# clintpgeorge/LDAGroupedGibbsSampler

Hardware: AMD Instinct MI355X
Metric: M tokens sampled/sec (whole node) per Gibbs sweep at K=100 (higher is better)
Workload: dtype f64

## Files before the change

### include/ggs_hip.h

```cpp
#ifndef GGS_HIP_H
#define GGS_HIP_H

#include <stdint.h>

#ifdef __cplusplus
extern "C" {
#endif

#define GGS_ABI_VERSION 6

typedef struct ggs_handle ggs_handle;

enum {
  GGS_OK = 0,
  GGS_ERR_NEGATIVE_COUNT = 1,
  GGS_ERR_INVALID_TOPIC = 2,
  GGS_ERR_RNG_EXHAUSTED = 3,
  GGS_ERR_BAD_ARG = 4,
  GGS_ERR_HIP = 5,
  GGS_ERR_STATE = 6,
  GGS_ERR_UNSUPPORTED = 7,
  GGS_ERR_INVARIANT = 8
};

// ... 47 lines not shown
  double exchange_ms;
  double exchange_rs_ms;
  double exchange_ag_ms;
} ggs_timings;

int ggs_create(const ggs_config *cfg, ggs_handle **out);
void ggs_destroy(ggs_handle *h);
const char *ggs_last_error(const ggs_handle *h);
int ggs_abi_version(void);
int ggs_set_stream(ggs_handle *h, void *hip_stream);

int ggs_set_corpus(ggs_handle *h, int64_t num_docs, const int64_t *doc_ptr ,
                   const int32_t *tokens , int64_t doc_base, int64_t tok_base);
int ggs_init_z_java_lcg(ggs_handle *h, int32_t seed);
int ggs_java_lcg_next_ints(int32_t seed, int32_t bound, int64_t n, int32_t *out);
int ggs_set_z(ggs_handle *h, const int32_t *z , int32_t redraw_phi);
int ggs_init_phi(ggs_handle *h);
int ggs_set_iteration(ggs_handle *h, int32_t iteration);
int ggs_get_iteration(const ggs_handle *h, int32_t *iteration);

int ggs_sweep(ggs_handle *h, int32_t n_sweeps);
int ggs_sweep_begin(ggs_handle *h);
int ggs_sweep_end(ggs_handle *h);
int ggs_sweep_end_async(ggs_handle *h);
int ggs_collapsed_serial_sweep(ggs_handle *h, int32_t java_seed, int32_t n_sweeps);
int ggs_sample_z_given_phi(ggs_handle *h, int32_t n_sweeps);
int ggs_counts_device_ptr(ggs_handle *h, void **dev_ptr, int64_t *num_elems);
int ggs_set_global_token_count(ggs_handle *h, int64_t n_tokens);
int ggs_synchronize(ggs_handle *h);

typedef struct ggs_exchange_ops {
  int32_t struct_size;
  int32_t reserved;
  void *ctx;
  int (*reduce_scatter_i32)(void *ctx, const void *send, void *recv, int64_t recv_count, void *hip_stream);
  int (*all_gather_f64)(void *ctx, const void *send, void *recv, int64_t send_count, void *hip_stream);
  int (*all_gather_i32)(void *ctx, const void *send, void *recv, int64_t send_count, void *hip_stream);
  int (*all_to_all_v_i32)(void *ctx, const void *send, const int64_t *send_offsets, const int64_t *send_counts, void *recv,
                          const int64_t *recv_offsets, const int64_t *recv_counts, void *hip_stream);
} ggs_exchange_ops;
#define GGS_EXCHANGE_OPS_V3_SIZE ((int32_t)(sizeof(ggs_exchange_ops) - sizeof(void *)))
int ggs_attach_exchange(ggs_handle *h, int32_t rank, int32_t nranks, const ggs_exchange_ops *ops);
#define GGS_RCCL_UNIQUE_ID_BYTES 128
int ggs_rccl_unique_id(void *out_id );
int ggs_attach_rccl(ggs_handle *h, int32_t rank, int32_t nranks, const void *unique_id);
int ggs_attach_rccl_comm(ggs_handle *h, int32_t rank, int32_t nranks, void *nccl_comm);
int ggs_group_create(const ggs_config *cfg, int32_t n, const int32_t *device_ids, ggs_handle **out_handles );
void ggs_group_destroy(ggs_handle **handles, int32_t n);
int ggs_group_set_z(ggs_handle **handles, int32_t n, const int32_t *const *z , int32_t redraw_phi);
int ggs_group_sweep(ggs_handle **handles, int32_t n, int32_t n_sweeps);
int ggs_group_adopt(ggs_handle **handles, int32_t n);
int ggs_group_gather_counts(ggs_handle **handles, int32_t n);
int ggs_attach_null_exchange(ggs_handle *h, int32_t rank, int32_t nranks);
int ggs_set_count_exchange(ggs_handle *h, int32_t mode);
int ggs_get_count_exchange(const ggs_handle *h, int32_t *sparse, int64_t *pairs_last, int64_t *cells);
int ggs_get_exchange_info(const ggs_handle *h, int32_t *rank, int32_t *nranks, int32_t *k_begin, int32_t *k_end);
int ggs_get_exchange_provider(const ggs_handle *h, int32_t *provider, int32_t *comm_nranks, int32_t *comm_rank);

int ggs_get_z(ggs_handle *h, int32_t *z );
int ggs_get_type_topic_counts(ggs_handle *h, int32_t *n_wk );
int ggs_get_topic_totals(ggs_handle *h, int32_t *n_k );
int ggs_get_phi(ggs_handle *h, double *phi );
int ggs_set_phi(ggs_handle *h, const double *phi );
int ggs_get_phi_mean(ggs_handle *h, double *phi_mean , int32_t *n_sampled);
int ggs_get_theta(ggs_handle *h, int64_t doc_begin, int64_t doc_end, double *theta );
int ggs_get_doc_topic_counts(ggs_handle *h, int64_t doc_begin, int64_t doc_end, int32_t *n_dk);
int ggs_get_timings(ggs_handle *h, ggs_timings *out);

int ggs_doc_topic_histogram(ggs_handle *h, int32_t symmetric, int64_t n_bins, int32_t *hist, int32_t *doc_lengths);
int ggs_type_topic_count_histogram(ggs_handle *h, int64_t n_bins, int32_t *hist);
int ggs_set_hyperparameters(ggs_handle *h, const double *alpha, double beta, double beta_sum);
int ggs_get_hyperparameters(const ggs_handle *h, double *alpha , double *beta, double *beta_sum);
int ggs_learn_symmetric_concentration(const int32_t *count_hist, int64_t n_hist, const int32_t *obs_lengths, int64_t n_len,
                                      int32_t num_dimensions, double current, double *out);
int ggs_learn_parameters(double *params , int32_t K, const int32_t *obs , int64_t n_bins,
                         const int32_t *obs_lengths, int64_t n_len, double shape, double scale, int32_t iterations, double *sum_out);
int ggs_reset_timings(ggs_handle *h);
int ggs_check_invariants(ggs_handle *h);
int ggs_get_launch_info(ggs_handle *h, int64_t *num_chunks, int32_t *lds_bytes_z, int32_t *docs_per_block_theta);
int ggs_get_num_hot_words(ggs_handle *h, int32_t *num_hot);
int ggs_get_warm_tiers(ggs_handle *h, int32_t *tiers, int32_t *warm_words, int32_t *docs_per_chunk);
int ggs_get_z_parts(ggs_handle *h, int32_t *parts);
int ggs_get_z_form(ggs_handle *h, int32_t *kernel, int32_t *form, int32_t *calibrated);
int ggs_debug_philox(int32_t device_id, int64_t n, const uint32_t *ctr , const uint32_t *key , uint32_t *out );
int ggs_debug_math(int32_t device_id, int32_t op , int64_t n, const double *x, const double *y, double *out);
int ggs_debug_draw(int32_t device_id, int32_t kind , uint64_t seed, uint32_t iteration,
                   uint32_t purpose, uint64_t elem0, int64_t n, const double *shape, double *out, int32_t *status);
int ggs_debug_poisson(int32_t device_id, double beta, int32_t threshold, uint64_t seed, uint32_t iteration, uint32_t purpose, uint64_t elem0,
                      int64_t n, const int32_t *counts, int32_t *out);
int ggs_debug_alias(int32_t device_id, int32_t V, int32_t K, const double *phi, const double *alpha, double *ps, int32_t *a, double *type_norm);
int ggs_get_alias_tables(ggs_handle *h, double *ps , int32_t *a , double *type_norm );
int ggs_set_topic_priors(ggs_handle *h, int64_t n_zero, const int32_t *topic, const int32_t *word);
int ggs_get_topic_priors(ggs_handle *h, double *priors );
int ggs_get_mh_stats(ggs_handle *h, int64_t out[3]);
int ggs_get_word_topic_lists(ggs_handle *h, int32_t *nw , int32_t *topics );
int ggs_get_sparse_stats(ggs_handle *h, int64_t out[4]);
int ggs_set_variable_selection_prior(ggs_handle *h, double pi);
int ggs_get_vs_stats(ggs_handle *h, int64_t out[3]);
int ggs_debug_vs_indicators(int32_t device_id, int32_t V, int32_t K, const int32_t *counts, const double *prev_phi, double beta, double pi, uint64_t seed,
                            uint32_t iteration, const double *u , uint8_t *drawn_out, int32_t *s_end, int32_t *rounds);
int ggs_model_log_likelihood(ggs_handle *h, double *doc_side, double *topic_side);
int ggs_log_posterior(ggs_handle *h, double *doc_side, double *topic_side);
int ggs_min_doc_distances(ggs_handle *h, const double *other , int64_t n_other, double *min_dist );
int ggs_min_topic_distance(ggs_handle *h, double *min_dist);
#define GGS_TOP_WORDS 0
#define GGS_TOP_RELEVANCE 1
#define GGS_TOP_DISTINCTIVE 2
#define GGS_TOP_SALIENT 3
#define GGS_TOP_K1 4
#define GGS_TOP_WORDS_MAX 128
int ggs_top_words(ggs_handle *h, int32_t kind, int32_t n_words, double lambda, int32_t *idx , double *score );
#define GGS_TOPIC_DIAGNOSTICS_MAX_TOPICS 3072
#define GGS_TOPIC_SCORE_ROWS 10
#define GGS_TOPIC_WORD_SCORE_ROWS 4
int ggs_topic_doc_statistics(ggs_handle *h, int32_t n_words, const int32_t *idx , const double *clogc_in ,
                             int32_t *codoc , int32_t *doc_stats , double *clogc_out );
int ggs_topic_scores(ggs_handle *h, int32_t n_words, const int32_t *idx , const int32_t *codoc, const int32_t *doc_stats,
                     const double *clogc, double *topic_scores , double *word_scores );
int ggs_set_test_corpus(ggs_handle *h, int64_t D, const int64_t *doc_ptr , const int32_t *tokens, int64_t doc_base);
int ggs_heldout_log_likelihood(ggs_handle *h, int32_t num_particles, double *doc_ll, double *total);
int ggs_debug_column_sum(int32_t device_id, int32_t V, int32_t K, const double *x , const int32_t *counts ,
                         double beta, double *out );
int ggs_debug_column_sum_guided(int32_t device_id, int32_t V, int32_t K, const double *x, const int32_t *counts, double beta,
                                const double *guess, double *out, double *pref_out, int32_t *n_k_out);
int ggs_debug_min_distances(int32_t device_id, const double *a, int64_t n, const double *b , int64_t m, int64_t len, int32_t element_major,
                            double *min_dist , double *min_sq );
int ggs_debug_topic_summaries(int32_t device_id, int32_t V, int32_t K, const int32_t *counts , double beta, double lambda, int32_t kind,
                              int32_t n_words, int32_t *idx , double *score , double *mass_k ,
                              double *rowsum_w , double *total , double *all_scores );
int ggs_debug_top_words_phases(ggs_handle *h, int32_t kind, int32_t n_words, double lambda, int32_t element_chain, double *ms );

int ggs_debug_topic_doc_statistics(int32_t device_id, int64_t D, const int64_t *doc_ptr, const int32_t *tokens, const int32_t *z, int32_t V, int32_t K,
                                   const double *alpha , int32_t n_words, const int32_t *idx, const double *clogc_in , int32_t *codoc,
                                   int32_t *doc_stats, double *clogc_out);
int ggs_debug_topic_scores(int32_t device_id, int32_t V, int32_t K, const int32_t *counts , double beta, int32_t n_words, const int32_t *idx,
                           const int32_t *codoc, const int32_t *doc_stats, const double *clogc, double *topic_scores, double *word_scores ,
                           int32_t *sorted_ids );
int ggs_debug_topic_diagnostics_phases(ggs_handle *h, int32_t n_words, double *ms );
#ifdef __cplusplus
}
#endif
#endif
```

### ldagroupedgibbssampler_amd/_lib.py

```python
import ctypes as C
import os
import subprocess

_HERE = os.path.dirname(os.path.abspath(__file__))
CSRC = os.path.join(_HERE, "csrc")
LIB_PATH = os.environ.get("GGS_HIP_LIB") or os.path.join(CSRC, "libggs_hip.so")
HEADER_PATH = os.path.join(os.path.dirname(_HERE), "include", "ggs_hip.h")

ABI_VERSION = 6


class GGSConfig(C.Structure):
    _fields_ = [
        ("struct_size", C.c_int32),
        ("num_topics", C.c_int32),
        ("num_types", C.c_int32),
        ("device_id", C.c_int32),
        ("alpha", C.POINTER(C.c_double)),
        ("alpha_scalar", C.c_double),
        ("beta", C.c_double),
        ("seed", C.c_uint64),
        ("flags", C.c_int32),
        ("phi_burn_in", C.c_int32),
        ("phi_mean_thin", C.c_int32),
        ("alias_poisson_threshold", C.c_int32),
    ]


class GGSTimings(C.Structure):
    _fields_ = [
        ("theta_ms", C.c_double),
        ("z_ms", C.c_double),
        ("merge_ms", C.c_double),
        ("phi_ms", C.c_double),
        ("sweeps", C.c_int64),
        ("tokens_sampled", C.c_int64),
        ("exchange_ms", C.c_double),
        ("exchange_rs_ms", C.c_double),
        ("exchange_ag_ms", C.c_double),
    ]


EXCHANGE_CB = C.CFUNCTYPE(C.c_int, C.c_void_p, C.c_void_p, C.c_void_p, C.c_int64, C.c_void_p)


A2AV_CB = C.CFUNCTYPE(C.c_int, C.c_void_p, C.c_void_p, C.POINTER(C.c_int64), C.POINTER(C.c_int64), C.c_void_p, C.POINTER(C.c_int64), C.POINTER(C.c_int64),
                      C.c_void_p)


class GGSExchangeOps(C.Structure):
    _fields_ = [
        ("struct_size", C.c_int32),
        ("reserved", C.c_int32),
        ("ctx", C.c_void_p),
        ("reduce_scatter_i32", EXCHANGE_CB),
        ("all_gather_f64", EXCHANGE_CB),
        ("all_gather_i32", EXCHANGE_CB),
        ("all_to_all_v_i32", A2AV_CB),
    ]


_vp = C.c_void_p
_dp = C.POINTER(C.c_double)
_ip = C.POINTER(C.c_int32)
_lp = C.POINTER(C.c_int64)
_up = C.POINTER(C.c_uint32)

SIGNATURES = {
    "ggs_create": (C.c_int, [C.POINTER(GGSConfig), C.POINTER(_vp)]),
    "ggs_destroy": (None, [_vp]),
    "ggs_last_error": (C.c_char_p, [_vp]),
    "ggs_abi_version": (C.c_int, []),
    "ggs_set_stream": (C.c_int, [_vp, _vp]),
    "ggs_set_corpus": (C.c_int, [_vp, C.c_int64, _lp, _ip, C.c_int64, C.c_int64]),
    "ggs_init_z_java_lcg": (C.c_int, [_vp, C.c_int32]),
    "ggs_java_lcg_next_ints": (C.c_int, [C.c_int32, C.c_int32, C.c_int64, _ip]),
    "ggs_set_z": (C.c_int, [_vp, _ip, C.c_int32]),
    "ggs_init_phi": (C.c_int, [_vp]),
    "ggs_set_iteration": (C.c_int, [_vp, C.c_int32]),
    "ggs_get_iteration": (C.c_int, [_vp, _ip]),
    "ggs_sweep": (C.c_int, [_vp, C.c_int32]),
    "ggs_sweep_begin": (C.c_int, [_vp]),
    "ggs_sweep_end": (C.c_int, [_vp]),
    "ggs_sweep_end_async": (C.c_int, [_vp]),
    "ggs_sample_z_given_phi": (C.c_int, [_vp, C.c_int32]),
    "ggs_collapsed_serial_sweep": (C.c_int, [_vp, C.c_int32, C.c_int32]),
    "ggs_counts_device_ptr": (C.c_int, [_vp, C.POINTER(_vp), _lp]),
    "ggs_set_global_token_count": (C.c_int, [_vp, C.c_int64]),
    "ggs_synchronize": (C.c_int, [_vp]),
    "ggs_get_z": (C.c_int, [_vp, _ip]),
    "ggs_get_type_topic_counts": (C.c_int, [_vp, _ip]),
    "ggs_get_topic_totals": (C.c_int, [_vp, _ip]),
    "ggs_get_phi": (C.c_int, [_vp, _dp]),
    "ggs_set_phi": (C.c_int, [_vp, _dp]),
    "ggs_get_phi_mean": (C.c_int, [_vp, _dp, _ip]),
    "ggs_get_theta": (C.c_int, [_vp, C.c_int64, C.c_int64, _dp]),
    "ggs_get_doc_topic_counts": (C.c_int, [_vp, C.c_int64, C.c_int64, _ip]),
    "ggs_get_timings": (C.c_int, [_vp, C.POINTER(GGSTimings)]),
    "ggs_reset_timings": (C.c_int, [_vp]),
    "ggs_check_invariants": (C.c_int, [_vp]),
    "ggs_get_launch_info": (C.c_int, [_vp, _lp, _ip, _ip]),
    "ggs_get_num_hot_words": (C.c_int, [_vp, _ip]),
    "ggs_get_z_parts": (C.c_int, [_vp, _ip]),
    "ggs_get_z_form": (C.c_int, [_vp, _ip, _ip, _ip]),
    "ggs_get_warm_tiers": (C.c_int, [_vp, _ip, _ip, _ip]),
    "ggs_attach_exchange": (C.c_int, [_vp, C.c_int32, C.c_int32, C.POINTER(GGSExchangeOps)]),
    "ggs_rccl_unique_id": (C.c_int, [_vp]),
    "ggs_attach_rccl": (C.c_int, [_vp, C.c_int32, C.c_int32, _vp]),
    "ggs_attach_rccl_comm": (C.c_int, [_vp, C.c_int32, C.c_int32, _vp]),
    "ggs_group_create": (C.c_int, [C.POINTER(GGSConfig), C.c_int32, _ip, C.POINTER(_vp)]),
    "ggs_group_destroy": (None, [C.POINTER(_vp), C.c_int32]),
    "ggs_group_adopt": (C.c_int, [C.POINTER(_vp), C.c_int32]),
    "ggs_group_set_z": (C.c_int, [C.POINTER(_vp), C.c_int32, C.POINTER(_ip), C.c_int32]),
    "ggs_group_sweep": (C.c_int, [C.POINTER(_vp), C.c_int32, C.c_int32]),
    "ggs_group_gather_counts": (C.c_int, [C.POINTER(_vp), C.c_int32]),
    "ggs_attach_null_exchange": (C.c_int, [_vp, C.c_int32, C.c_int32]),
    "ggs_get_exchange_info": (C.c_int, [_vp, _ip, _ip, _ip, _ip]),
    "ggs_get_exchange_provider": (C.c_int, [_vp, _ip, _ip, _ip]),
    "ggs_set_count_exchange": (C.c_int, [_vp, C.c_int32]),
    "ggs_get_count_exchange": (C.c_int, [_vp, _ip, _lp, _lp]),
    "ggs_debug_philox": (C.c_int, [C.c_int32, C.c_int64, _up, _up, _up]),
    "ggs_debug_math": (C.c_int, [C.c_int32, C.c_int32, C.c_int64, _dp, _dp, _dp]),
    "ggs_debug_draw": (C.c_int, [C.c_int32, C.c_int32, C.c_uint64, C.c_uint32, C.c_uint32, C.c_uint64, C.c_int64,
                                 _dp, _dp, _ip]),
    "ggs_debug_poisson": (C.c_int, [C.c_int32, C.c_double, C.c_int32, C.c_uint64, C.c_uint32, C.c_uint32, C.c_uint64, C.c_int64, _ip, _ip]),
    "ggs_debug_alias": (C.c_int, [C.c_int32, C.c_int32, C.c_int32, _dp, _dp, _dp, _ip, _dp]),
    "ggs_get_alias_tables": (C.c_int, [_vp, _dp, _ip, _dp]),
    "ggs_set_topic_priors": (C.c_int, [_vp, C.c_int64, _ip, _ip]),
    "ggs_get_topic_priors": (C.c_int, [_vp, _dp]),
    "ggs_get_mh_stats": (C.c_int, [_vp, _lp]),
    "ggs_get_word_topic_lists": (C.c_int, [_vp, _ip, _ip]),
    "ggs_get_sparse_stats": (C.c_int, [_vp, _lp]),
    "ggs_set_variable_selection_prior": (C.c_int, [_vp, C.c_double]),
    "ggs_get_vs_stats": (C.c_int, [_vp, _lp]),
    "ggs_debug_vs_indicators": (C.c_int, [C.c_int32, C.c_int32, C.c_int32, _ip, _dp, C.c_double, C.c_double, C.c_uint64, C.c_uint32, _dp,
                                          C.POINTER(C.c_uint8), _ip, _ip]),
    "ggs_doc_topic_histogram": (C.c_int, [_vp, C.c_int32, C.c_int64, _ip, _ip]),
    "ggs_type_topic_count_histogram": (C.c_int, [_vp, C.c_int64, _ip]),
    "ggs_set_hyperparameters": (C.c_int, [_vp, _dp, C.c_double, C.c_double]),
    "ggs_get_hyperparameters": (C.c_int, [_vp, _dp, _dp, _dp]),
    "ggs_learn_symmetric_concentration": (C.c_int, [_ip, C.c_int64, _ip, C.c_int64, C.c_int32, C.c_double, _dp]),
    "ggs_learn_parameters": (C.c_int, [_dp, C.c_int32, _ip, C.c_int64, _ip, C.c_int64, C.c_double, C.c_double, C.c_int32, _dp]),
    "ggs_model_log_likelihood": (C.c_int, [_vp, _dp, _dp]),
    "ggs_log_posterior": (C.c_int, [_vp, _dp, _dp]),
    "ggs_min_doc_distances": (C.c_int, [_vp, _dp, C.c_int64, _dp]),
    "ggs_min_topic_distance": (C.c_int, [_vp, _dp]),
    "ggs_top_words": (C.c_int, [_vp, C.c_int32, C.c_int32, C.c_double, _ip, _dp]),
    "ggs_topic_doc_statistics": (C.c_int, [_vp, C.c_int32, _ip, _dp, _ip, _ip, _dp]),
    "ggs_topic_scores": (C.c_int, [_vp, C.c_int32, _ip, _ip, _ip, _dp, _dp, _dp]),
    "ggs_set_test_corpus": (C.c_int, [_vp, C.c_int64, _lp, _ip, C.c_int64]),
    "ggs_heldout_log_likelihood": (C.c_int, [_vp, C.c_int32, _dp, _dp]),
    "ggs_debug_column_sum": (C.c_int, [C.c_int32, C.c_int32, C.c_int32, _dp, _ip, C.c_double, _dp]),
    "ggs_debug_column_sum_guided": (C.c_int, [C.c_int32, C.c_int32, C.c_int32, _dp, _ip, C.c_double, _dp, _dp, _dp, _ip]),
    "ggs_debug_min_distances": (C.c_int, [C.c_int32, _dp, C.c_int64, _dp, C.c_int64, C.c_int64, C.c_int32, _dp, _dp]),
    "ggs_debug_top_words_phases": (C.c_int, [_vp, C.c_int32, C.c_int32, C.c_double, C.c_int32, _dp]),
    "ggs_debug_topic_doc_statistics": (C.c_int, [C.c_int32, C.c_int64, _lp, _ip, _ip, C.c_int32, C.c_int32, _dp, C.c_int32, _ip, _dp, _ip, _ip, _dp]),
    "ggs_debug_topic_scores": (C.c_int, [C.c_int32, C.c_int32, C.c_int32, _ip, C.c_double, C.c_int32, _ip, _ip, _ip, _dp, _dp, _dp, _ip]),
    "ggs_debug_topic_diagnostics_phases": (C.c_int, [_vp, C.c_int32, _dp]),
    "ggs_debug_topic_summaries": (C.c_int, [C.c_int32, C.c_int32, C.c_int32, _ip, C.c_double, C.c_double, C.c_int32, C.c_int32, _ip, _dp, _dp, _dp, _dp, _dp]),
}


def build(force=False):
    srcs = [os.path.join(CSRC, f) for f in os.listdir(CSRC) if f.endswith((".hip", ".hpp"))] + [HEADER_PATH]
    if (not force and os.path.exists(LIB_PATH)
            and all(os.path.getmtime(LIB_PATH) >= os.path.getmtime(s) for s in srcs)):
        return LIB_PATH
    subprocess.check_call(["make", "-C", CSRC, "libggs_hip.so"])
    return LIB_PATH


_lib = None


def _share_hip_runtime_with_torch():
    import importlib.util
    import sys
    if "torch" in sys.modules:
        return
    try:
        spec = importlib.util.find_spec("torch")
    except (ImportError, ValueError):
        return
    if spec is None or not spec.origin:
        return
    cand = os.path.join(os.path.dirname(spec.origin), "lib", "libamdhip64.so")
    if os.path.exists(cand):
        C.CDLL(cand, mode=C.RTLD_GLOBAL)
# ... 35 lines not shown
```

### ldagroupedgibbssampler_amd/csrc/ggs_api.hip

```cpp
#include "ggs_host_state.hpp"
#include "ggs_host_plan.hpp"
#include "ggs_host_counts.hpp"
#include "ggs_host_phi.hpp"
#include "ggs_host_sweep.hpp"
#include "ggs_host_exchange.hpp"
#include "ggs_host_end_of_run.hpp"
#include "ggs_host_hyper.hpp"
#include "ggs_host_debug.hpp"

extern "C" {

int ggs_abi_version(void) { return GGS_ABI_VERSION; }

const char *ggs_last_error(const ggs_handle *h) { return h ? h->err.c_str() : "null handle"; }

int ggs_create(const ggs_config *cfg, ggs_handle **out) {
  if (!cfg || !out) return GGS_ERR_BAD_ARG;
  *out = nullptr;
  if (cfg->struct_size != (int32_t)sizeof(ggs_config)) return GGS_ERR_BAD_ARG;
  if (cfg->num_topics <= 0 || cfg->num_types <= 0 || !(cfg->beta > 0)) return GGS_ERR_BAD_ARG;
  Scheme scheme = Scheme::ggs; int32_t poisson_L = 0;
  if (const int rc = scheme_of(cfg, scheme, poisson_L)) return rc;
  int ndev = 0;
  if (hipGetDeviceCount(&ndev) != hipSuccess || ndev <= 0 || cfg->device_id < 0 || cfg->device_id >= ndev) return GGS_ERR_HIP;
// ... 67 lines not shown
  }
  if (poisson_phi(h->scheme)) {
    std::vector<double> T;
    build_poisson_table(h->beta, h->pa_L, T);
    h->pa_t00 = T[0];
    if ((rc = upload(h, &h->d_pa_table, T)) || (rc = dev_alloc(h, &h->d_pa_acc, (size_t)h->K * kPoissonAccStride))) return bail(rc);
  }
  if (count_tables(h->scheme) && (rc = dev_alloc_zeroed(h, &h->d_tpt, (size_t)h->V))) return bail(rc);
  if (h->scheme == Scheme::adlda && ((rc = dev_alloc_zeroed(h, &h->d_ad_den0, (size_t)h->K)) || (rc = dev_alloc_zeroed(h, &h->d_ad_s0, 1)))) return bail(rc);
  if (h->scheme == Scheme::collapsed && (rc = dev_alloc(h, &h->d_lcg, 2))) return bail(rc);
  for (auto &e : h->ev_part)
    if (make_event(h, &e, hipEventDisableTiming)) return bail(GGS_ERR_HIP);
  for (auto &E : h->evs)
    for (hipEvent_t *e : {&E.e[0], &E.e[1], &E.e[2], &E.e[3], &E.e[4], &E.e[5], &E.x[0], &E.x[1], &E.x[2], &E.th0, &E.th1})
      if (make_event(h, e)) return bail(GGS_ERR_HIP);
  {
    int lo = 0, hi = 0;
    (void)hipDeviceGetStreamPriorityRange(&lo, &hi);
    if (make_stream(h, &h->side, lo) || make_stream(h, &h->side_hot, hi) || make_event(h, &h->ev_hot_fork) || make_event(h, &h->ev_hot_join) ||
        make_event(h, &h->ev_chain_done, hipEventDisableTiming))
      return bail(GGS_ERR_HIP);
  }
  if (hipDeviceSynchronize() != hipSuccess) return bail(GGS_ERR_HIP);
  *out = h;
  return GGS_OK;
}

void ggs_destroy(ggs_handle *h) {
  if (!h) return;
  (void)hipSetDevice(h->device);
  (void)hipDeviceSynchronize();
  if (h->d_replays) {
    unsigned long long n = 0;
    if (hipMemcpy(&n, h->d_replays, sizeof(n), hipMemcpyDeviceToHost) == hipSuccess)
      fprintf(stderr, "[ggs] z replays: %llu tokens in %lld launches of z_sliced32_kernel (%.2f per launch)\n", n, (long long)h->z_f32_launches,
              h->z_f32_launches ? (double)n / (double)h->z_f32_launches : 0.0);
  }
  for (void **slot : h->owned)
    if (*slot) (void)hipFree(*slot);
  if (h->d_scratch) (void)hipFree(h->d_scratch);
  if (h->d_heldout_spill) (void)hipFree(h->d_heldout_spill);
  exchange_free(h->xg);
  for (hipStream_t st : h->owned_streams) (void)hipStreamDestroy(st);
  for (hipEvent_t ev : h->owned_events) (void)hipEventDestroy(ev);
  delete h;
}

int ggs_set_stream(ggs_handle *h, void *hip_stream) {
  if (!h) return GGS_ERR_BAD_ARG;
  int rc = bind_device(h);
  if (rc) return rc;
  HIP_TRY(h, hipStreamSynchronize(h->stream));
  if ((rc = drop_theta_ahead(h))) return rc;
  if (h->xg && !hip_stream) return set_err(h, GGS_ERR_BAD_ARG, "with an exchange attached the handle does not run on the legacy default stream");
  h->stream = reinterpret_cast<hipStream_t>(hip_stream);
  return GGS_OK;
}

int ggs_set_corpus(ggs_handle *h, int64_t D, const int64_t *doc_ptr, const int32_t *tokens, int64_t doc_base, int64_t tok_base) {
  if (!h || D < 0 || !doc_ptr || doc_base < 0 || tok_base < 0) return set_err(h, GGS_ERR_BAD_ARG, "bad corpus arguments");
  if (doc_ptr[0] != 0) return set_err(h, GGS_ERR_BAD_ARG, "doc_ptr[0] must be 0");
  for (int64_t d = 0; d < D; ++d)
    if (doc_ptr[d + 1] < doc_ptr[d]) return set_err(h, GGS_ERR_BAD_ARG, "doc_ptr must be non-decreasing");
  const int64_t N = doc_ptr[D];
  if (N > 0 && !tokens) return set_err(h, GGS_ERR_BAD_ARG, "tokens is null");
  if (N >= (int64_t)1 << 31 || D >= (int64_t)1 << 31) return set_err(h, GGS_ERR_UNSUPPORTED, "more than 2^31-1 tokens or documents per device");
  for (int64_t i = 0; i < N; ++i)
    if (tokens[i] < 0 || tokens[i] >= h->V) return set_err(h, GGS_ERR_BAD_ARG, "token id outside [0, num_types)");
  int rc = bind_device(h);
  if (rc) return rc;
  if ((rc = drop_theta_ahead(h))) return rc;

  const LaunchPlan &pl = h->plan;
  int32_t parts = pl.cfg_parts.parts;
  if (!pl.parts_forced && parts > 1) parts = D <= (int64_t)h->V ? 1 : D < 2 * (int64_t)h->V ? std::min(parts, 4) : parts;
  h->cfg = parts > 1 ? &pl.cfg_parts : &pl.cfg_plain;

  const bool pcgs = pcgs_family(h->scheme);
  CorpusShape shape;
  shape.V = h->V; shape.tile_tokens = pl.tile_tokens; shape.z_parts = parts;
  shape.pcgs = pcgs; shape.sliced = pl.sliced(); shape.two_rows = pl.two_rows;
  shape.hot_cap = pl.hot_cap; shape.warm_cap = pl.warm_cap; shape.warm_docs = pl.warm_docs;
  shape.warm_tiers_max = pl.warm_tiers_max; shape.warm_min_fill_pct = pl.warm_min_fill_pct; shape.warm_min_chunks_per_wave = pl.warm_min_chunks_per_wave;
  shape.sliced_waves = (int64_t)h->num_cus * kSlicedWaves; shape.pcgs_waves = (int64_t)h->num_cus * pl.lane.per_cu;
  const CorpusLists L = build_corpus_lists(shape, D, doc_ptr, tokens);
  if (pcgs) {
    h->pcgs_wave = pl.wave_forced || L.longest > kPcgsMaxDocLen;
    if (h->pcgs_wave && !pl.wave.fn) return set_err(h, GGS_ERR_UNSUPPORTED, "scheme=pcgs: a document of 32768 tokens or more with more than 4096 topics");
    h->pcgs_z = pcgs_entry(pl, h->scheme, h->pcgs_wave);
    h->pcgs_items = (wave_only(h->scheme) || h->pcgs_wave) ? (int64_t)L.order.size() : ((int64_t)L.order.size() + 63) / 64;
    if (const auto corpus_lds = row_of(h->scheme).corpus_lds) {
      h->sp_cap = (int32_t)std::max<int64_t>(1, std::min<int64_t>(h->K, L.longest));
      h->pcgs_z.lds = (int)corpus_lds(h->K, h->sp_cap);
      h->pcgs_z.per_cu = h->scheme == Scheme::spalias ? lds_workgroups_per_cu(h->pcgs_z.lds, 32) : resident_waves_per_cu(h->pcgs_z.fn, h->pcgs_z.lds);
      if (const char *e = debug_env("GGS_DEBUG_SPALIAS_WPC")) h->pcgs_z.per_cu = std::max(1, std::min(h->pcgs_z.per_cu, std::atoi(e)));
    }
  }
  h->D = D; h->N = N; h->C = (int64_t)L.cstart.size(); h->S = (int64_t)L.seg_word.size(); h->doc_base = doc_base; h->tok_base = tok_base;
  h->part_doc = L.part_doc; h->part_chunk = L.part_chunk;
  h->pcgs_order_len = (int64_t)L.order.size();
  h->num_hot = (int32_t)L.hot_words.size(); h->HS = (int64_t)L.hseg_word.size();
  h->Cc = L.Cc; h->Cs = L.Cs;
  h->warm_tiers = L.warm_tiers; h->num_warm = L.num_warm; h->Cw = L.Cw; h->warm_chunks_max = L.warm_chunks_max; h->warm_rows_max = L.warm_rows_max;

  const size_t theta_elems = (size_t)D * h->K + 2;
  if ((rc = upload(h, &h->d_doc_ptr, doc_ptr, (size_t)D + 1)) || (rc = upload(h, &h->d_tok, tokens, (size_t)N)) ||
      (rc = upload(h, &h->d_perm, L.perm)) || (rc = upload(h, &h->d_inv_perm, L.inv)) ||
      (rc = upload(h, &h->d_seg_word, L.seg_word)) || (rc = upload(h, &h->d_seg_begin, L.seg_begin)))
    return rc;
  if (pcgs && (rc = upload(h, &h->d_order, L.order))) return rc;
  if (pl.sliced() && ((rc = upload(h, &h->d_ct_tok, L.ct_tok)) || (rc = upload(h, &h->d_ct_idx, L.ct_idx)) || (rc = upload(h, &h->d_ct_ip, L.ct_ip)) ||
                      (rc = upload(h, &h->d_c_docs, L.c_docs)) || (rc = upload(h, &h->d_hot_words, L.hot_words)) ||
                      (rc = upload(h, &h->d_ht_pack, L.ht_pack)) || (rc = upload(h, &h->d_h_docs, L.h_docs)) ||
                      (rc = upload(h, &h->d_hseg_word, L.hseg_word)) || (rc = upload(h, &h->d_hseg_begin, L.hseg_begin)) || (rc = upload(h, &h->d_hseg_end, L.hseg_end))))
    return rc;
  if (h->C && ((rc = upload(h, &h->d_chunk_start, L.cstart)) || (rc = upload(h, &h->d_chunk_doc, L.cdoc)) || (rc = upload(h, &h->d_chunk_len, L.clen)) ||
               (pl.two_rows && (rc = upload(h, &h->d_chunk_doc1, L.cdoc1)))))
    return rc;
  if (L.warm_tiers > 0 && ((rc = upload(h, &h->d_wt_pack, L.wt_pack)) || (rc = upload(h, &h->d_w_docs, L.w_docs)) ||
                           (rc = upload(h, &h->d_warm_words, L.warm_words)) || (rc = upload(h, &h->d_warm_meta, L.warm_meta))))
    return rc;
  const bool with_theta = !counts_only(h->scheme) && !no_theta(h->scheme);
  if (!with_theta && h->d_theta) { (void)hipFree(h->d_theta); h->d_theta = nullptr; }
  if ((rc = dev_alloc(h, &h->d_z, (size_t)N)) || (rc = dev_alloc(h, &h->d_zw, (size_t)N)) ||
      (with_theta && (rc = dev_alloc(h, &h->d_theta, theta_elems))) || (!pcgs && (rc = dev_alloc(h, &h->d_theta_next, theta_elems))))
    return rc;
  HIP_TRY(h, hipMemset(h->d_z, 0, sizeof(int32_t) * std::max<size_t>((size_t)N, 1)));
  HIP_TRY(h, hipMemset(h->d_zw, 0, sizeof(int32_t) * std::max<size_t>((size_t)N, 1)));
  if (with_theta) HIP_TRY(h, hipMemset(h->d_theta, 0, sizeof(double) * std::max<size_t>((size_t)D * h->K, 1)));
  if (!pcgs) HIP_TRY(h, hipMemset(h->d_theta_next, 0, sizeof(double) * std::max<size_t>((size_t)D * h->K, 1)));
  if (h->d_mh) HIP_TRY(h, hipMemset(h->d_mh, 0, 3 * sizeof(unsigned long long)));
  if (h->d_ps_stats) HIP_TRY(h, hipMemset(h->d_ps_stats, 0, 4 * sizeof(unsigned long long)));
  if (h->d_phi_mean) HIP_TRY(h, hipMemset(h->d_phi_mean, 0, sizeof(double) * (size_t)h->K * h->V));
  h->n_sampled_phi = 0;
  HIP_TRY(h, hipDeviceSynchronize());

  h->have_corpus = true; h->have_phi = false; h->in_sweep = false; h->global_tokens = -1; h->lcg_ready = false;
  h->z_split = pl.split; h->z_split_tried = pl.split_forced;
  h->counts_global = h->xg == nullptr; h->cnt_own_valid = false; h->n_k_valid = false;
  return GGS_OK;
}

int ggs_init_z_java_lcg(ggs_handle *h, int32_t seed) {
  int rc = require_ready(h, false);
  if (rc) return rc;
  if (h->tok_base != 0) return set_err(h, GGS_ERR_STATE, "java-LCG init is one sequential stream: only valid with tok_base == 0");
  if ((rc = drop_theta_ahead(h))) return rc;
  std::vector<int32_t> z((size_t)h->N);
  const uint64_t lcg_state = java_lcg_next_ints(seed, h->K, h->N, z.data());
  if (h->scheme == Scheme::collapsed) {
    HIP_TRY(h, hipMemcpyAsync(h->d_lcg, &lcg_state, sizeof lcg_state, hipMemcpyHostToDevice, h->stream));
    h->lcg_ready = true;
  }
  if (h->N) HIP_TRY(h, hipMemcpyAsync(h->d_z, z.data(), sizeof(int32_t) * (size_t)h->N, hipMemcpyHostToDevice, h->stream));
  if ((rc = launch_permute_z(h))) return rc;
  if ((rc = launch_count_rebuild(h))) return rc;
  HIP_TRY(h, hipStreamSynchronize(h->stream));
  return GGS_OK;
}

int ggs_set_z(ggs_handle *h, const int32_t *z, int32_t redraw_phi) {
  int rc = require_ready(h, false);
  if (rc) return rc;
  if (h->N > 0 && !z) return set_err(h, GGS_ERR_BAD_ARG, "z is null");
  for (int64_t i = 0; i < h->N; ++i)
    if (z[i] < 0 || z[i] >= h->K) return set_err(h, GGS_ERR_BAD_ARG, "topic indicator outside [0, num_topics)");
  if ((rc = drop_theta_ahead(h))) return rc;
  h->lcg_ready = false;
  if (h->N) HIP_TRY(h, hipMemcpyAsync(h->d_z, z, sizeof(int32_t) * (size_t)h->N, hipMemcpyHostToDevice, h->stream));
  if ((rc = launch_permute_z(h))) return rc;
  if ((rc = launch_count_rebuild(h))) return rc;
  HIP_TRY(h, hipStreamSynchronize(h->stream));
  if (redraw_phi) return ggs_init_phi(h);
  return GGS_OK;
}

int ggs_init_phi(ggs_handle *h) {
  int rc = require_ready(h, false);
  if (rc) return rc;
  if (count_form(h->scheme)) {
    if ((rc = launch_magnitude(h))) return rc;
    h->have_phi = true;
    return check_status(h);
  }
  if ((rc = launch_phi(h, true, false))) return rc;
  return check_status(h);
}

int ggs_set_iteration(ggs_handle *h, int32_t it) {
  if (!h) return GGS_ERR_BAD_ARG;
  if (it < 0) return set_err(h, GGS_ERR_BAD_ARG, "the iteration number is 0 ... INT32_MAX");
  h->iteration = it;
  return GGS_OK;
}
int ggs_get_iteration(const ggs_handle *h, int32_t *it) { if (!h || !it) return GGS_ERR_BAD_ARG; *it = h->iteration; return GGS_OK; }

bool chain_on_side_ok(const ggs_handle *h) {
  return h->theta_main && h->plan.sliced() && h->side_hot && h->ev_chain_done && !h->xg &&
         (h->D >= (int64_t)h->V || h->theta_main_always);
}

// ... 767 lines not shown
  }
  if ((rc = dev_alloc(h, &h->d_test_docs, (size_t)D))) return rc;
  {
    size_t at = 0;
    for (const std::vector<int32_t> *ids : {&h->test_short, &h->test_long, &h->test_huge}) {
      if (!ids->empty()) HIP_TRY(h, hipMemcpy(h->d_test_docs + at, ids->data(), sizeof(int32_t) * ids->size(), hipMemcpyHostToDevice));
      at += ids->size();
    }
  }
  h->test_doc_base = doc_base;
  h->have_test = true;
  return GGS_OK;
}

int ggs_heldout_log_likelihood(ggs_handle *h, int32_t num_particles, double *doc_ll, double *total) {
  int rc = require_ready(h, false);
  if (rc) return rc;
  if (!h->have_test) return set_err(h, GGS_ERR_STATE, "no test set: call ggs_set_test_corpus first");
  if (num_particles < 1 || !total) return set_err(h, GGS_ERR_BAD_ARG, "num_particles < 1 or null output");
  return heldout_evaluate(h, num_particles, doc_ll, total);
}

int ggs_get_timings(ggs_handle *h, ggs_timings *out) { if (!h || !out) return GGS_ERR_BAD_ARG; *out = h->tm; return GGS_OK; }
int ggs_reset_timings(ggs_handle *h) { if (!h) return GGS_ERR_BAD_ARG; h->tm = ggs_timings{}; return GGS_OK; }

int ggs_check_invariants(ggs_handle *h) {
  int rc = require_ready(h, false);
  if (rc) return rc;
  const int K = h->K;
  const size_t bytes = 16 + sizeof(int32_t) * (size_t)K;
  if ((rc = ensure_global_counts(h))) return rc;
  if ((rc = ensure_scratch(h, bytes))) return rc;
  auto *d_total = static_cast<unsigned long long *>(h->d_scratch);
  auto *d_flags = reinterpret_cast<uint32_t *>(static_cast<char *>(h->d_scratch) + 8);
  auto *d_col = reinterpret_cast<int32_t *>(static_cast<char *>(h->d_scratch) + 16);
  HIP_TRY(h, hipMemsetAsync(h->d_scratch, 0, bytes, h->stream));
  const int64_t kv = (int64_t)K * h->V;
  hipLaunchKernelGGL(invariants_kernel, dim3(grid_for(kv, 256)), dim3(256), 0, h->stream, h->d_n_wk, kv, K, d_total, d_col, d_flags);
  HIP_TRY(h, hipGetLastError());
  if ((rc = launch_magnitude(h))) return rc;
  std::vector<unsigned char> host(bytes);
  std::vector<int32_t> nk((size_t)K);
  if ((rc = copy_out(h, host.data(), h->d_scratch, bytes))) return rc;
  if ((rc = copy_out(h, nk.data(), h->d_n_k, sizeof(int32_t) * (size_t)K))) return rc;
  unsigned long long total; uint32_t fl;
  std::memcpy(&total, host.data(), 8); std::memcpy(&fl, host.data() + 8, 4);
  const int32_t *col = reinterpret_cast<const int32_t *>(host.data() + 16);
  if (fl & 1u) return set_err(h, GGS_ERR_INVARIANT, "negative type-topic count");
  if ((int64_t)total != (h->global_tokens >= 0 ? h->global_tokens : h->N)) return set_err(h, GGS_ERR_INVARIANT, "type-topic counts do not sum to the corpus size");
  for (int k = 0; k < K; ++k)
    if (col[k] != nk[(size_t)k]) return set_err(h, GGS_ERR_INVARIANT, "column sum differs from tokensPerTopic");
  return GGS_OK;
}

int ggs_get_launch_info(ggs_handle *h, int64_t *num_chunks, int32_t *lds_bytes_z, int32_t *docs_per_block_theta) {
  if (!h) return GGS_ERR_BAD_ARG;
  const LaunchPlan &pl = h->plan;
  const bool pcgs = pcgs_family(h->scheme);
  if (num_chunks) *num_chunks = pcgs ? h->pcgs_items : pl.sliced() ? h->Cs + h->Cw : h->C;
  if (lds_bytes_z) *lds_bytes_z = pcgs ? h->pcgs_z.lds : pl.sliced() ? sliced_fused_lds(h->K, pl.hot_cap) : pl.z.lds;
  if (docs_per_block_theta) *docs_per_block_theta = h->cfg->theta_docs;
  return GGS_OK;
}

int ggs_get_num_hot_words(ggs_handle *h, int32_t *num_hot) {
  if (!h || !num_hot) return GGS_ERR_BAD_ARG;
  *num_hot = h->plan.sliced() ? h->num_hot + h->num_warm : 0;
  return GGS_OK;
}

int ggs_get_z_parts(ggs_handle *h, int32_t *parts) {
  if (!h || !parts) return GGS_ERR_BAD_ARG;
  const int32_t P = (int32_t)h->part_doc.size() - 1;
  *parts = (h->plan.stream() && h->overlap_theta && P > 1) ? P : 1;
  return GGS_OK;
}

int ggs_get_warm_tiers(ggs_handle *h, int32_t *tiers, int32_t *warm_words, int32_t *docs_per_chunk) {
  if (!h) return GGS_ERR_BAD_ARG;
  const bool on = h->have_corpus && h->plan.sliced();
  if (tiers) *tiers = on ? h->warm_tiers : 0;
  if (warm_words) *warm_words = on ? h->num_warm : 0;
  if (docs_per_chunk) *docs_per_chunk = on && h->warm_tiers ? h->plan.warm_docs : 0;
  return GGS_OK;
}

int ggs_get_z_form(ggs_handle *h, int32_t *kernel, int32_t *form, int32_t *calibrated) {
  if (!h) return GGS_ERR_BAD_ARG;
  const bool splittable = h->plan.sliced() && h->Cs > h->Cc && h->Cc > 0;
  const int32_t own = row_of(h->scheme).z_kernel;
  if (kernel) *kernel = own ? own : pcgs_family(h->scheme) ? (h->pcgs_wave ? 5 : 4) : h->plan.kernel;
  if (form) *form = h->plan.sliced() ? (splittable && h->z_split ? 1 : 2) : 0;
  if (calibrated) *calibrated = (splittable && h->z_split_tried && !h->plan.split_forced && h->plan.split) ? 1 : 0;
  return GGS_OK;
}

int ggs_java_lcg_next_ints(int32_t seed, int32_t bound, int64_t n, int32_t *out) {
  if (bound <= 0 || n < 0 || (n > 0 && !out)) return GGS_ERR_BAD_ARG;
  java_lcg_next_ints(seed, bound, n, out);
  return GGS_OK;
}

int ggs_debug_philox(int32_t device_id, int64_t n, const uint32_t *ctr, const uint32_t *key, uint32_t *out) {
  if (n <= 0 || !ctr || !key || !out || hipSetDevice(device_id) != hipSuccess) return GGS_ERR_BAD_ARG;
  TmpDev t;
  auto *dc = static_cast<uint32_t *>(t.get(n * 16)); auto *dk = static_cast<uint32_t *>(t.get(n * 8)); auto *dou = static_cast<uint32_t *>(t.get(n * 16));
  if (!dc || !dk || !dou) return GGS_ERR_HIP;
  if (hipMemcpy(dc, ctr, n * 16, hipMemcpyHostToDevice) != hipSuccess || hipMemcpy(dk, key, n * 8, hipMemcpyHostToDevice) != hipSuccess) return GGS_ERR_HIP;
  hipLaunchKernelGGL(debug_philox_kernel, dim3((unsigned)((n + 255) / 256)), dim3(256), 0, nullptr, n, dc, dk, dou);
  if (hipMemcpy(out, dou, n * 16, hipMemcpyDeviceToHost) != hipSuccess) return GGS_ERR_HIP;
  return GGS_OK;
}

int ggs_debug_math(int32_t device_id, int32_t op, int64_t n, const double *x, const double *y, double *out) {
  if (n <= 0 || !x || !out || hipSetDevice(device_id) != hipSuccess) return GGS_ERR_BAD_ARG;
  TmpDev t;
  auto *dx = static_cast<double *>(t.get(n * 8)); auto *dy = static_cast<double *>(t.get(n * 8)); auto *dou = static_cast<double *>(t.get(n * 8));
  if (!dx || !dy || !dou) return GGS_ERR_HIP;
  if (hipMemcpy(dx, x, n * 8, hipMemcpyHostToDevice) != hipSuccess) return GGS_ERR_HIP;
  if (hipMemcpy(dy, y ? y : x, n * 8, hipMemcpyHostToDevice) != hipSuccess) return GGS_ERR_HIP;
  hipLaunchKernelGGL(debug_math_kernel, dim3((unsigned)((n + 255) / 256)), dim3(256), 0, nullptr, op, n, dx, dy, dou);
  if (hipMemcpy(out, dou, n * 8, hipMemcpyDeviceToHost) != hipSuccess) return GGS_ERR_HIP;
  return GGS_OK;
}

int ggs_debug_draw(int32_t device_id, int32_t kind, uint64_t seed, uint32_t iteration, uint32_t purpose, uint64_t elem0, int64_t n,
                   const double *shape, double *out, int32_t *status) {
  if (n <= 0 || !out || (kind == 2 && !shape) || hipSetDevice(device_id) != hipSuccess) return GGS_ERR_BAD_ARG;
  TmpDev t;
  auto *ds = static_cast<double *>(t.get(n * 8)); auto *dou = static_cast<double *>(t.get(n * 8)); auto *dst = static_cast<uint32_t *>(t.get(16));
  if (!ds || !dou || !dst) return GGS_ERR_HIP;
  if (shape && hipMemcpy(ds, shape, n * 8, hipMemcpyHostToDevice) != hipSuccess) return GGS_ERR_HIP;
  if (hipMemset(dst, 0, 16) != hipSuccess) return GGS_ERR_HIP;
  hipLaunchKernelGGL(debug_draw_kernel, dim3((unsigned)((n + 255) / 256)), dim3(256), 0, nullptr, kind, seed, iteration, purpose, elem0, n, ds, dou, dst);
  uint32_t st = 0;
  if (hipMemcpy(out, dou, n * 8, hipMemcpyDeviceToHost) != hipSuccess || hipMemcpy(&st, dst, 4, hipMemcpyDeviceToHost) != hipSuccess) return GGS_ERR_HIP;
  if (status) *status = (int32_t)st;
  return GGS_OK;
}

int ggs_debug_poisson(int32_t device_id, double beta, int32_t threshold, uint64_t seed, uint32_t iteration, uint32_t purpose, uint64_t elem0, int64_t n,
                      const int32_t *counts, int32_t *out) {
  const int32_t L = threshold == 0 ? 100 : threshold;
  if (n <= 0 || !counts || !out || !(beta > 0) || L < 1 || L > kPoissonMaxThreshold || hipSetDevice(device_id) != hipSuccess) return GGS_ERR_BAD_ARG;
  for (int64_t i = 0; i < n; ++i)
    if (counts[i] < 0) return GGS_ERR_BAD_ARG;
  std::vector<double> T;
  build_poisson_table(beta, L, T);
  TmpDev t;
  auto *dt = static_cast<double *>(t.get(T.size() * 8)); auto *dc = static_cast<int32_t *>(t.get(n * 4));
  auto *dou = static_cast<int32_t *>(t.get(n * 4)); auto *dst = static_cast<uint32_t *>(t.get(16));
  if (!dt || !dc || !dou || !dst) return GGS_ERR_HIP;
  if (hipMemcpy(dt, T.data(), T.size() * 8, hipMemcpyHostToDevice) != hipSuccess || hipMemcpy(dc, counts, n * 4, hipMemcpyHostToDevice) != hipSuccess ||
      hipMemset(dst, 0, 16) != hipSuccess)
    return GGS_ERR_HIP;
  hipLaunchKernelGGL(debug_poisson_kernel, dim3((unsigned)((n + 255) / 256)), dim3(256), 0, nullptr, seed, iteration, purpose, elem0, n, dc, L, beta, dt, T[0],
                     dou, dst);
  uint32_t st = 0;
  if (hipGetLastError() != hipSuccess || hipMemcpy(out, dou, n * 4, hipMemcpyDeviceToHost) != hipSuccess || hipMemcpy(&st, dst, 4, hipMemcpyDeviceToHost) != hipSuccess)
    return GGS_ERR_HIP;
  return st ? GGS_ERR_RNG_EXHAUSTED : GGS_OK;
}

int ggs_debug_alias(int32_t device_id, int32_t V, int32_t K, const double *phi, const double *alpha, double *ps, int32_t *a, double *type_norm) {
  if (V <= 0 || K <= 0 || K > kPcgsWaveMaxTopics || !phi || !alpha || !ps || !a || !type_norm || hipSetDevice(device_id) != hipSuccess) return GGS_ERR_BAD_ARG;
  const size_t kv = (size_t)K * V;
// ... 196 lines not shown
```

### ldagroupedgibbssampler_amd/csrc/ggs_corpus_lists.hpp

```cpp
#pragma once
#include <stdint.h>

#include <algorithm>
#include <utility>
#include <vector>

#include "ggs_layout.hpp"

namespace ggs {

struct CorpusShape {
  int32_t V = 0;
  bool pcgs = false;
  bool sliced = false;
  bool two_rows = false;
  int32_t tile_tokens = 64;
  int32_t z_parts = 1;
  int32_t hot_cap = 0, warm_cap = 0, warm_docs = 0;
  int32_t warm_tiers_max = 0, warm_min_fill_pct = 0, warm_min_chunks_per_wave = 0;
  int64_t sliced_waves = 0;
  int64_t pcgs_waves = 0;
};

struct CorpusLists {
  int64_t D = 0, N = 0;
  std::vector<int64_t> cstart;
  std::vector<int32_t> cdoc, clen, cdoc1;
  std::vector<int64_t> part_doc, part_chunk;
  std::vector<int32_t> perm, inv, seg_word, seg_begin, hot_words, hseg_word, hseg_begin, hseg_end;
  std::vector<int32_t> order;
  int64_t longest = 0;
  std::vector<int32_t> ct_tok, ct_idx, ct_ip, c_docs;
  int64_t Cc = 0, Cs = 0;
  std::vector<int32_t> ht_pack, h_docs;
  int32_t warm_tiers = 0, num_warm = 0, warm_rows_max = 0;
  int64_t Cw = 0, warm_chunks_max = 0;
  std::vector<int32_t> wt_pack, w_docs, warm_words;
  std::vector<int64_t> warm_meta;
};

namespace lists_detail {

struct ChunkBuilder {
  int maxdocs = kChunkDocs, docslots = kChunkDocs, shift = kSlotShift;
  std::vector<int32_t> tok, idx, docs;
  int fill = 64, ndocs = 0, last = -1;
  int64_t tokens = 0;
  void add(int32_t value, int32_t token, int32_t doc) {
    if (fill == 64 || (doc != last && ndocs == maxdocs)) {
      tok.resize(tok.size() + 64, 0); idx.resize(idx.size() + 64, -1);
      docs.insert(docs.end(), (size_t)docslots, doc);
      fill = 0; ndocs = 1; last = doc;
    } else if (doc != last) {
      docs[docs.size() - (size_t)docslots + (size_t)ndocs] = doc; ++ndocs; last = doc;
    }
    const size_t at = tok.size() - 64 + (size_t)fill;
    tok[at] = value | ((ndocs - 1) << shift); idx[at] = token;
    ++fill; ++tokens;
  }
  int64_t chunks() const { return (int64_t)(tok.size() / 64); }
  void sort_lanes() {
    std::vector<std::pair<uint32_t, int32_t>> tmp(64);
    for (size_t c0 = 0; c0 < tok.size(); c0 += 64) {
      int n = 0;
      while (n < 64 && idx[c0 + (size_t)n] >= 0) ++n;
      for (int j = 0; j < n; ++j) tmp[(size_t)j] = {(uint32_t)tok[c0 + (size_t)j], idx[c0 + (size_t)j]};
      std::sort(tmp.begin(), tmp.begin() + n);
      for (int j = 0; j < n; ++j) { tok[c0 + (size_t)j] = (int32_t)tmp[(size_t)j].first; idx[c0 + (size_t)j] = tmp[(size_t)j].second; }
    }
  }
};

inline void chunk_table(const CorpusShape &s, const int64_t D, const int64_t *doc_ptr, CorpusLists &L) {
  const int64_t N = L.N;
  L.cstart.reserve((size_t)(N / 48 + D)); L.cdoc.reserve(L.cstart.capacity()); L.clen.reserve(L.cstart.capacity());
  if (s.two_rows) {
    int64_t pos = 0, d = 0;
    while (pos < N) {
      while (doc_ptr[d + 1] <= pos) ++d;
      const int64_t take0 = std::min<int64_t>(64, doc_ptr[d + 1] - pos);
      int64_t len = take0, d1 = d;
      if (take0 < 64 && pos + take0 < N) {
        d1 = d + 1;
        while (doc_ptr[d1 + 1] <= pos + take0) ++d1;
        len += std::min<int64_t>(64 - take0, doc_ptr[d1 + 1] - (pos + take0));
      }
      L.cstart.push_back(pos); L.cdoc.push_back((int32_t)d); L.cdoc1.push_back((int32_t)d1);
      L.clen.push_back((int32_t)(len | (take0 << 8)));
      pos += len;
    }
    return;
  }
  for (int64_t d = 0; d < D; ++d) {
    const int64_t len = doc_ptr[d + 1] - doc_ptr[d];
    if (len == 0) continue;
    const int64_t T = s.tile_tokens, n = (len + T - 1) / T, base = len / n, rem = len % n;
    int64_t at = doc_ptr[d];
    for (int64_t j = 0; j < n; ++j) {
      const int64_t l = base + (j < rem ? 1 : 0);
      L.cstart.push_back(at); L.cdoc.push_back((int32_t)d); L.clen.push_back((int32_t)l);
      at += l;
    }
  }
}

inline void z_parts(const CorpusShape &s, const int64_t D, const int64_t *doc_ptr, CorpusLists &L) {
  const int32_t P = (s.z_parts > 1 && D >= 64 * s.z_parts) ? s.z_parts : 1;
  const int64_t C = (int64_t)L.cstart.size();
  L.part_doc.assign((size_t)P + 1, D); L.part_chunk.assign((size_t)P + 1, C);
  L.part_doc[0] = 0; L.part_chunk[0] = 0;
  int64_t d = 0;
  size_t c = 0;
  for (int32_t p = 1; p < P; ++p) {
    const int64_t want = L.N * p / P;
    while (d < D && doc_ptr[d] < want) ++d;
    while (c < L.cdoc.size() && L.cdoc[c] < d) ++c;
    L.part_doc[(size_t)p] = d; L.part_chunk[(size_t)p] = (int64_t)c;
  }
}

inline std::vector<int32_t> word_order(const CorpusShape &s, const int32_t *tokens, CorpusLists &L) {
  const int64_t N = L.N;
  std::vector<int32_t> warm_cand;
  L.perm.resize((size_t)N); L.inv.resize((size_t)N);
  std::vector<int64_t> wptr((size_t)s.V + 1, 0);
  for (int64_t i = 0; i < N; ++i) wptr[(size_t)tokens[i] + 1]++;
  for (int32_t w = 0; w < s.V; ++w) wptr[(size_t)w + 1] += wptr[(size_t)w];
  for (int32_t w = 0; w < s.V; ++w)
    for (int64_t b = wptr[(size_t)w]; b < wptr[(size_t)w + 1]; b += kSegTokens) { L.seg_word.push_back(w); L.seg_begin.push_back((int32_t)b); }
  L.seg_begin.push_back((int32_t)N);
  std::vector<int64_t> cur(wptr.begin(), wptr.end() - 1);
  for (int64_t i = 0; i < N; ++i) L.perm[(size_t)cur[(size_t)tokens[i]]++] = (int32_t)i;
  for (int64_t i = 0; i < N; ++i) L.inv[(size_t)L.perm[(size_t)i]] = (int32_t)i;
  if (s.sliced && !s.pcgs && s.hot_cap > 0) {
    std::vector<int32_t> order((size_t)s.V);
    for (int32_t w = 0; w < s.V; ++w) order[(size_t)w] = w;
    const size_t nh = (size_t)std::min<int32_t>(s.hot_cap, s.V);
    const size_t nw = std::min<size_t>((size_t)s.V, nh + (size_t)s.warm_tiers_max * (size_t)s.warm_cap);
    auto freq = [&](int32_t w) { return wptr[(size_t)w + 1] - wptr[(size_t)w]; };
    std::partial_sort(order.begin(), order.begin() + nw, order.end(), [&](int32_t a, int32_t b) { return freq(a) != freq(b) ? freq(a) > freq(b) : a < b; });
    for (size_t r = 0; r < nh && freq(order[r]) > 0; ++r) L.hot_words.push_back(order[r]);
    for (size_t r = nh; r < nw && freq(order[r]) > 0; ++r) warm_cand.push_back(order[r]);
    for (int32_t w : L.hot_words)
      for (int64_t b = wptr[(size_t)w]; b < wptr[(size_t)w + 1]; b += kSegTokens) {
        L.hseg_word.push_back(w); L.hseg_begin.push_back((int32_t)b); L.hseg_end.push_back((int32_t)std::min(b + kSegTokens, wptr[(size_t)w + 1]));
      }
  }
  return warm_cand;
}

inline void pcgs_order(const CorpusShape &s, const int64_t D, const int64_t *doc_ptr, CorpusLists &L) {
  std::vector<int32_t> &order = L.order;
  order.resize((size_t)D);
  for (int64_t d = 0; d < D; ++d) { order[(size_t)d] = (int32_t)d; L.longest = std::max(L.longest, doc_ptr[d + 1] - doc_ptr[d]); }
  std::stable_sort(order.begin(), order.end(), [&](int32_t a, int32_t b) { return doc_ptr[a + 1] - doc_ptr[a] > doc_ptr[b + 1] - doc_ptr[b]; });
  const int64_t n_groups = (D + 63) / 64, W = s.pcgs_waves;
  if (n_groups > W && n_groups <= 2 * W) {
    const int64_t m = n_groups - W;
    std::vector<int32_t> padded((size_t)(2 * W * 64), -1);
    auto put = [&](int64_t position, int64_t group) {
      for (int64_t j = 0; j < 64 && group * 64 + j < D; ++j) padded[(size_t)(position * 64 + j)] = order[(size_t)(group * 64 + j)];
    };
    for (int64_t g = 0; g < W; ++g) put(g, g);
    for (int64_t j = 0; j < m; ++j) put(W + (W - m + j), n_groups - 1 - j);
    order.swap(padded);
  }
}

inline std::vector<int32_t> pack_lanes(const std::vector<int32_t> &tok, const std::vector<int32_t> &idx, const std::vector<int32_t> &inv) {
  std::vector<int32_t> pack(4 * idx.size(), 0);
  for (size_t j = 0; j < idx.size(); ++j) {
    pack[4 * j] = tok[j]; pack[4 * j + 1] = idx[j];
    if (idx[j] >= 0) pack[4 * j + 2] = inv[(size_t)idx[j]];
  }
  return pack;
}

inline void sliced_lists(const CorpusShape &s, const int64_t D, const int64_t *doc_ptr, const int32_t *tokens, std::vector<int32_t> warm_cand, CorpusLists &L) {
  ChunkBuilder cold, hot;
  std::vector<int32_t> row_of((size_t)s.V, -1);
  for (size_t r = 0; r < L.hot_words.size(); ++r) row_of[(size_t)L.hot_words[r]] = (int32_t)r;
  std::vector<ChunkBuilder> warm;
  int32_t tiers = 0;
  if (s.warm_cap > 0 && L.hot_words.size() == (size_t)s.hot_cap && !warm_cand.empty()) {
    const int32_t cand_tiers = (int32_t)((warm_cand.size() + (size_t)s.warm_cap - 1) / (size_t)s.warm_cap);
    warm.resize((size_t)cand_tiers);
    for (ChunkBuilder &b : warm) { b.maxdocs = s.warm_docs; b.docslots = kWarmDocSlots; b.shift = kWarmSlotShift; }
    std::vector<int32_t> warm_of((size_t)s.V, -1);
    for (size_t r = 0; r < warm_cand.size(); ++r) warm_of[(size_t)warm_cand[r]] = (int32_t)r;
    for (int64_t d = 0; d < D; ++d)
      for (int64_t i = doc_ptr[d]; i < doc_ptr[d + 1]; ++i) {
        const int32_t r = warm_of[(size_t)tokens[i]];
        if (r >= 0) warm[(size_t)(r / s.warm_cap)].add(r % s.warm_cap, (int32_t)i, (int32_t)d);
      }
    const int64_t min_chunks = (int64_t)s.warm_min_chunks_per_wave * s.sliced_waves;
    while (tiers < cand_tiers && warm[(size_t)tiers].tokens > 0 && warm[(size_t)tiers].chunks() >= min_chunks &&
           warm[(size_t)tiers].tokens * 100 >= warm[(size_t)tiers].chunks() * 64 * s.warm_min_fill_pct)
      ++tiers;
    warm.resize((size_t)tiers);
    warm_cand.resize(std::min(warm_cand.size(), (size_t)tiers * (size_t)s.warm_cap));
    for (int32_t w : warm_cand) row_of[(size_t)w] = -2;
  }
  for (int64_t d = 0; d < D; ++d)
    for (int64_t i = doc_ptr[d]; i < doc_ptr[d + 1]; ++i) {
      const int32_t r = row_of[(size_t)tokens[i]];
      if (r >= 0) hot.add(r, (int32_t)i, (int32_t)d);
      else if (r == -1) cold.add(tokens[i], (int32_t)i, (int32_t)d);
    }
  cold.sort_lanes();
  hot.sort_lanes();
  for (ChunkBuilder &b : warm) b.sort_lanes();
  L.Cc = cold.chunks();
  L.Cs = L.Cc + hot.chunks();
  {
    std::vector<int32_t> htok(hot.tok.size());
    for (size_t j = 0; j < htok.size(); ++j) {
      const uint32_t t = (uint32_t)hot.tok[j];
      htok[j] = (int32_t)((t & ((1u << kSlotShift) - 1)) | ((t >> kSlotShift) << kWarmSlotShift));
    }
    L.ht_pack = pack_lanes(htok, hot.idx, L.inv);
    L.h_docs.assign((size_t)hot.chunks() * (size_t)kWarmDocSlots, 0);
    for (size_t c = 0; c < (size_t)hot.chunks(); ++c)
      for (int r = 0; r < kWarmDocSlots; ++r) L.h_docs[c * (size_t)kWarmDocSlots + (size_t)r] = hot.docs[(size_t)kChunkDocs * c + (size_t)std::min(r, kChunkDocs - 1)];
  }
  L.ct_tok = std::move(cold.tok); L.ct_idx = std::move(cold.idx); L.c_docs = std::move(cold.docs);
  L.ct_tok.insert(L.ct_tok.end(), hot.tok.begin(), hot.tok.end());
  L.ct_idx.insert(L.ct_idx.end(), hot.idx.begin(), hot.idx.end());
  L.c_docs.insert(L.c_docs.end(), hot.docs.begin(), hot.docs.end());
  L.ct_ip.assign(L.ct_idx.size(), 0);
  for (size_t j = 0; j < L.ct_ip.size(); ++j)
    if (L.ct_idx[j] >= 0) L.ct_ip[j] = L.inv[(size_t)L.ct_idx[j]];
  L.warm_tiers = tiers; L.num_warm = (int32_t)warm_cand.size();
  if (tiers > 0) {
    std::vector<int32_t> wtok, widx;
    L.warm_words.assign((size_t)tiers * (size_t)s.warm_cap, 0);
    L.warm_meta.assign((size_t)(2 * tiers + 1), 0);
    for (int32_t t = 0; t < tiers; ++t) {
      const ChunkBuilder &b = warm[(size_t)t];
      L.warm_meta[(size_t)t] = (int64_t)(wtok.size() / 64);
      const int32_t rows = (int32_t)std::min<size_t>((size_t)s.warm_cap, warm_cand.size() - (size_t)t * (size_t)s.warm_cap);
      L.warm_meta[(size_t)(tiers + 1 + t)] = rows;
      L.warm_rows_max = std::max(L.warm_rows_max, rows);
      L.warm_chunks_max = std::max(L.warm_chunks_max, b.chunks());
      wtok.insert(wtok.end(), b.tok.begin(), b.tok.end());
      widx.insert(widx.end(), b.idx.begin(), b.idx.end());
      L.w_docs.insert(L.w_docs.end(), b.docs.begin(), b.docs.end());
      for (int32_t r = 0; r < rows; ++r) L.warm_words[(size_t)t * (size_t)s.warm_cap + (size_t)r] = warm_cand[(size_t)t * (size_t)s.warm_cap + (size_t)r];
    }
    L.warm_meta[(size_t)tiers] = (int64_t)(wtok.size() / 64);
    L.Cw = L.warm_meta[(size_t)tiers];
    L.wt_pack = pack_lanes(wtok, widx, L.inv);
  }
}

}

inline CorpusLists build_corpus_lists(const CorpusShape &s, const int64_t D, const int64_t *doc_ptr, const int32_t *tokens) {
  CorpusLists L;
  L.D = D; L.N = doc_ptr[D];
  std::vector<int32_t> warm_cand = lists_detail::word_order(s, tokens, L);
  if (s.pcgs) {
    lists_detail::pcgs_order(s, D, doc_ptr, L);
  } else if (s.sliced) {
    lists_detail::sliced_lists(s, D, doc_ptr, tokens, std::move(warm_cand), L);
  } else {
    lists_detail::chunk_table(s, D, doc_ptr, L);
    lists_detail::z_parts(s, D, doc_ptr, L);
  }
  return L;
}

}
```

### ldagroupedgibbssampler_amd/csrc/ggs_host_plan.hpp

```cpp
#pragma once
#include "ggs_host_state.hpp"

namespace {
#define GGS_KMAX_SWITCH(KERNEL)                                                                                                     \
  switch ((K + 7) / 8) {                                                                                                            \
    case 1: return reinterpret_cast<const void *>(KERNEL<8>);      case 2: return reinterpret_cast<const void *>(KERNEL<16>);       \
    case 3: return reinterpret_cast<const void *>(KERNEL<24>);     case 4: return reinterpret_cast<const void *>(KERNEL<32>);       \
    case 5: return reinterpret_cast<const void *>(KERNEL<40>);     case 6: return reinterpret_cast<const void *>(KERNEL<48>);       \
    case 7: return reinterpret_cast<const void *>(KERNEL<56>);     case 8: return reinterpret_cast<const void *>(KERNEL<64>);       \
    case 9: return reinterpret_cast<const void *>(KERNEL<72>);     case 10: return reinterpret_cast<const void *>(KERNEL<80>);      \
    case 11: return reinterpret_cast<const void *>(KERNEL<88>);    case 12: return reinterpret_cast<const void *>(KERNEL<96>);      \
    case 13: return reinterpret_cast<const void *>(KERNEL<104>);   case 14: return reinterpret_cast<const void *>(KERNEL<112>);     \
    case 15: return reinterpret_cast<const void *>(KERNEL<120>);   case 16: return reinterpret_cast<const void *>(KERNEL<128>);     \
    case 17: return reinterpret_cast<const void *>(KERNEL<136>);   case 18: return reinterpret_cast<const void *>(KERNEL<144>);     \
    case 19: return reinterpret_cast<const void *>(KERNEL<152>);   case 20: return reinterpret_cast<const void *>(KERNEL<160>);     \
    case 21: return reinterpret_cast<const void *>(KERNEL<168>);   case 22: return reinterpret_cast<const void *>(KERNEL<176>);     \
    case 23: return reinterpret_cast<const void *>(KERNEL<184>);   default: return reinterpret_cast<const void *>(KERNEL<192>);     \
  }
const void *sliced_kernel_for(int K) { GGS_KMAX_SWITCH(z_sliced_kernel) }
const void *sliced32_kernel_for(int K) { GGS_KMAX_SWITCH(z_sliced32_kernel) }

const void *hot_kernel_for(int K) { GGS_KMAX_SWITCH(z_hot_kernel) }
const void *warm_kernel_for(int K) { GGS_KMAX_SWITCH(z_warm_kernel) }
const void *pcgs_kernel_for(int K) { GGS_KMAX_SWITCH(pcgs_sliced_kernel) }
const void *polyaurn_kernel_for(int K) { GGS_KMAX_SWITCH(polyaurn_sliced_kernel) }
const void *collapsed_kernel_for(int K) {
  switch ((K + 7) / 8) {
#define GGS_CK(N) case N: return reinterpret_cast<const void *>(pcgs_sliced_kernel<8 * N, true>);
    GGS_CK(1) GGS_CK(2) GGS_CK(3) GGS_CK(4) GGS_CK(5) GGS_CK(6) GGS_CK(7) GGS_CK(8) GGS_CK(9) GGS_CK(10) GGS_CK(11) GGS_CK(12)
    GGS_CK(13) GGS_CK(14) GGS_CK(15) GGS_CK(16) GGS_CK(17) GGS_CK(18) GGS_CK(19) GGS_CK(20) GGS_CK(21) GGS_CK(22) GGS_CK(23)
#undef GGS_CK
    default: return reinterpret_cast<const void *>(pcgs_sliced_kernel<192, true>);
  }
}

const void *pcgs_wave_kernel_for(int nb, bool collapsed, bool polyaurn) {
#define GGS_WK(N) if (nb <= N) return polyaurn ? reinterpret_cast<const void *>(polyaurn_wave_kernel<N>) : collapsed ? reinterpret_cast<const void *>(pcgs_wave_kernel<N, true>) : reinterpret_cast<const void *>(pcgs_wave_kernel<N, false>);
  GGS_WK(1) GGS_WK(2) GGS_WK(4) GGS_WK(8) GGS_WK(16)
#undef GGS_WK
  return polyaurn ? reinterpret_cast<const void *>(polyaurn_wave_kernel<32>) : collapsed ? reinterpret_cast<const void *>(pcgs_wave_kernel<32, true>) : reinterpret_cast<const void *>(pcgs_wave_kernel<32, false>);
}
constexpr int kPcgsWaveMaxTopics = 32 * 128;
constexpr int kPcgsWaveFromTopics = 176, kCollapsedWaveFromTopics = 96;
constexpr int kPolyaurnWaveFromTopics = 168;

const void *tile_kernel_for(int K) {
  const int nt = (K + 63) / 64;
  return nt <= 1 ? reinterpret_cast<const void *>(z_kernel<1>) : nt <= 2 ? reinterpret_cast<const void *>(z_kernel<2>)
       : nt <= 4 ? reinterpret_cast<const void *>(z_kernel<4>) : nt <= 8 ? reinterpret_cast<const void *>(z_kernel<8>)
       : nt <= 16 ? reinterpret_cast<const void *>(z_kernel<16>) : reinterpret_cast<const void *>(z_kernel<20>);
}
const void *stream_kernel_for(bool two_pass, bool regck, int group) {
  if (two_pass) return reinterpret_cast<const void *>(z_stream_kernel);
  if (!regck) return reinterpret_cast<const void *>(z_stream1_kernel<false, 4>);
  return group == 1 ? reinterpret_cast<const void *>(z_stream1_kernel<true, 1>) : group == 2 ? reinterpret_cast<const void *>(z_stream1_kernel<true, 2>)
                                                                                             : reinterpret_cast<const void *>(z_stream1_kernel<true, 4>);
}
const void *pcgs_lane_kernel_for(int K, bool sliced, bool collapsed, bool polyaurn) {
  if (sliced) return collapsed ? collapsed_kernel_for(K) : polyaurn ? polyaurn_kernel_for(K) : pcgs_kernel_for(K);
  return collapsed ? reinterpret_cast<const void *>(pcgs_z_kernel<true>) : polyaurn ? reinterpret_cast<const void *>(polyaurn_z_kernel) : reinterpret_cast<const void *>(pcgs_z_kernel<false>);
}

int resident_waves_per_cu(const void *fn, int lds) {
  int by_regs = 0;
  if (hipOccupancyMaxActiveBlocksPerMultiprocessor(&by_regs, fn, 64, (size_t)lds) != hipSuccess || by_regs < 1) by_regs = 1;
  return lds_workgroups_per_cu(lds, std::min(by_regs, 32));
}

int plan_launches(const int K, const int V, const Scheme scheme, const Knobs &kn, LaunchPlan &pl) {
  const int Kp = (K + 1) & ~1, pitch16 = (Kp / 2) | 1;
  if (doc_hist_lds_bytes(K) <= (size_t)kMaxLdsBytes) {
    pl.dochist = {reinterpret_cast<const void *>(doc_topic_hist_kernel), kHistBlock, (int)doc_hist_lds_bytes(K), 0};
    pl.dochist.per_cu = lds_workgroups_per_cu(pl.dochist.lds, kHistPerCu);
  }
  pl.cellhist = {reinterpret_cast<const void *>(cell_hist_kernel), kHistBlock, kCellHistLdsBytes, kHistPerCu};
  if (scheme == Scheme::ggs) {
    const bool sliced_ok = K <= kSlicedMaxTopics && V < (1 << kSlotShift);
    bool sliced = sliced_ok && K <= kSlicedDefaultTopics, stream = !sliced && K > 2 * kSliceTopics, two_pass = false;
    if (kn.zkernel.set) {
      const int mode = kn.zkernel.v;
      sliced = sliced_ok && mode == 1;
      stream = (mode == 2 || mode == 3) ? K > 2 * kSliceTopics : (stream && mode != 0);
      two_pass = mode == 3;
      if (sliced) stream = false;
    }
    pl.kernel = sliced ? 1 : stream ? (two_pass ? 3 : 2) : 0;
    if (stream) {
      const int ns = stream_slices(K);
      int group = ns <= kRegCheckpoints ? 1 : ns <= 2 * kRegCheckpoints ? 2 : 4;
      if (kn.group.set && (kn.group.v == 1 || kn.group.v == 2 || kn.group.v == 4)) group = kn.group.v;
      bool regck = !two_pass && z_stream1_groups(K, group) <= kRegCheckpoints;
      if (kn.regck.set) regck = regck && kn.regck.v != 0;
      if (!regck) group = 4;
      pl.two_rows = !two_pass && (kn.tworows.set ? kn.tworows.v != 0 : K <= 512);
      pl.z.fn = stream_kernel_for(two_pass, regck, group);
      pl.z.lds = two_pass ? z_stream_lds_bytes(K) : z_stream1_lds_bytes(K, group, pl.two_rows, regck);
      if (pl.z.lds > kMaxLdsBytes) return GGS_ERR_UNSUPPORTED;
    } else if (sliced) {
      pl.f32 = !kn.phi64.is(1);
      pl.Kp32 = round_up(K, kSlice32Topics);
      pl.ring_base = sliced_ring_base(K); pl.wave_lds = sliced_wave_lds(K); pl.hot_pitch = table_row_pitch(K);
      pl.hot_wave_lds = hot_wave_lds(K); pl.warm_wave_lds = warm_wave_lds(K);
      if (kn.split.set) { pl.split = kn.split.v != 0; pl.split_forced = kn.split.v == 2; }
      pl.hot_cap = pl.split ? table_rows_beside_cold(K, pl.hot_wave_lds) : table_rows_fused(K);
      if (kn.hot.set) pl.hot_cap = std::max(0, std::min(pl.hot_cap, kn.hot.v));
      pl.cold = {pl.f32 ? sliced32_kernel_for(K) : sliced_kernel_for(K), kSlicedWaves * 64, sliced_cold_lds(K), 1};
      pl.hot = {hot_kernel_for(K), kSlicedWaves * 64, table_lds(K, pl.hot_wave_lds, 0), 1};
      pl.warm = {warm_kernel_for(K), kSlicedWaves * 64, table_lds(K, pl.warm_wave_lds, 0), 1};
      pl.warm_docs = warm_docs_for(sliced_kmax(K));
      pl.warm_cap = table_rows_beside_cold(K, pl.warm_wave_lds);
      if (pl.warm_cap < 16) pl.warm_cap = 0;
      if (kn.warm.set) pl.warm_tiers_max = std::max(0, std::min(kWarmMaxTiers, kn.warm.v));
      if (kn.warm_rows.set) pl.warm_cap = std::max(0, std::min(pl.warm_cap, kn.warm_rows.v));
      if (kn.warm_fill.set) pl.warm_min_fill_pct = std::max(1, std::min(100, kn.warm_fill.v));
      if (kn.warm_cpw.set) pl.warm_min_chunks_per_wave = std::max(0, kn.warm_cpw.v);
    } else {
      int T = z_tile_rows_in(kMaxLdsBytes / 6 / kLdsGranule * kLdsGranule, Kp, pitch16);
      if (kn.tile.set) T = kn.tile.v;
      pl.tile_tokens = std::max(8, std::min(64, T));
      pl.z.fn = tile_kernel_for(K);
      pl.z.lds = z_tile_lds_bytes(Kp, pitch16, pl.tile_tokens);
      if (pl.z.lds > kMaxLdsBytes) return GGS_ERR_UNSUPPORTED;
    }
    if (!sliced) {
      pl.z.per_cu = lds_workgroups_per_cu(pl.z.lds, 8);
      if (kn.wpc.set) pl.z.per_cu = std::max(1, kn.wpc.v);
    }
  }
  const int theta_quarter = (kMaxLdsBytes - 24 * 1024) / 4;
  int B = 64;
  while (B > 1 && (theta_cells_lds_bytes(K, B) > 32 * 1024 || (B > 16 && theta_lds_bytes(K, B) > theta_quarter))) B >>= 1;
  if (theta_lds_bytes(K, B) > kMaxLdsBytes) return GGS_ERR_UNSUPPORTED;
  pl.theta.fn = reinterpret_cast<const void *>(theta_kernel<kThetaBlock>); pl.theta.block = kThetaBlock;
  pl.cfg_plain = {1, pl.z.per_cu, B, std::max(theta_lds_bytes(K, B), theta_quarter), 0};
  pl.theta_docs_main = kn.theta_b.set ? std::max(1, std::min(B, kn.theta_b.v)) : std::min(B, 16);
  pl.theta_lds_main = std::max(theta_lds_bytes(K, pl.theta_docs_main), (kMaxLdsBytes - 24 * 1024) / (kn.theta_wgs.set ? std::max(1, kn.theta_wgs.v) : 5));
  pl.cfg_parts = pl.cfg_plain;
  if (scheme == Scheme::ggs) {
    pl.parts_forced = kn.zparts.set;
    int parts = kn.zparts.set ? std::max(1, std::min(8, kn.zparts.v)) : pl.kernel == 2 ? 8 : 1;
    if (parts > 1 && pl.kernel == 2) {
      const int kBeside = kn.beside.set ? std::max(1, kn.beside.v) : 4;
      const int z_alloc = lds_alloc_of(pl.z.lds);
      auto z_waves_beside = [&](int theta_lds) { return std::min(pl.z.per_cu, (kMaxLdsBytes - kLdsGranule - kBeside * lds_alloc_of(theta_lds)) / z_alloc); };
      int Bt = 64;
      while (Bt > 1 && theta_cells_lds_bytes(K, Bt) > 10 * 1024) Bt >>= 1;
      const int zw = z_waves_beside(theta_cells_lds_bytes(K, Bt));
      const int t_lds = theta_lds_bytes(K, Bt);
      if (theta_cells_lds_bytes(K, Bt) <= 12 * 1024 && zw >= 2)
        pl.cfg_parts = {parts, zw, Bt, std::max(t_lds, theta_quarter), std::max(t_lds, (kMaxLdsBytes - kLdsGranule - zw * z_alloc) / kBeside / kLdsGranule * kLdsGranule)};
      else
        parts = 1;
    }
    pl.cfg_parts.parts = parts;
    return GGS_OK;
  }

  const bool collapsed = scheme == Scheme::collapsed, polyaurn = scheme == Scheme::polyaurn;
  if (K <= kPcgsWaveMaxTopics) {
    const int nb = pcgs_wave_blocks(Kp);
    pl.wave.fn = pcgs_wave_kernel_for(nb, collapsed, polyaurn);
    pl.wave.lds = pcgs_wave_lds_bytes(nb);
    pl.wave.per_cu = resident_waves_per_cu(pl.wave.fn, pl.wave.lds);
  }
  pl.wave_forced = kn.pcgs_wave.set ? kn.pcgs_wave.v != 0 : K > (collapsed ? kCollapsedWaveFromTopics : polyaurn ? kPolyaurnWaveFromTopics : kPcgsWaveFromTopics);
  if (pl.wave_forced && !pl.wave.fn) return GGS_ERR_UNSUPPORTED;
  const bool lane_sliced = K <= kSlicedMaxTopics && !(kn.pcgs_stream.set && kn.pcgs_stream.v != 0);
  pl.lane.lds = lane_sliced ? pcgs_sliced_lds_bytes(K) : pcgs_z_lds_bytes(K);
  if (pl.lane.lds > kMaxLdsBytes && !pl.wave_forced) return GGS_ERR_UNSUPPORTED;
  pl.lane.per_cu = lds_workgroups_per_cu(pl.lane.lds, 8);
  if (!pl.wave_forced) pl.lane.fn = pcgs_lane_kernel_for(K, lane_sliced, collapsed, polyaurn);
  if (collapsed) pl.serial.fn = reinterpret_cast<const void *>(collapsed_serial_kernel);
  if (has_alias(scheme)) {
    pl.alias_wpb = alias_words_per_block(K);
    pl.alias = {reinterpret_cast<const void *>(alias_build_kernel), 64, (int)alias_lds_bytes(K, pl.alias_wpb), 0};
    pl.alias.per_cu = lds_workgroups_per_cu(pl.alias.lds, 16);
  }
  if (doubly_sparse(scheme)) pl.wordlist = {reinterpret_cast<const void *>(word_list_build_kernel), kWordListBlock, 0, 8};
  if (scheme == Scheme::spalias) pl.spalias.fn = reinterpret_cast<const void *>(spalias_wave_kernel);
  if (scheme == Scheme::polyaurn_sparse) pl.pusparse.fn = reinterpret_cast<const void *>(polyaurn_sparse_wave_kernel);
  if (scheme == Scheme::nzvsspalias) {
    pl.wordmask = {reinterpret_cast<const void *>(word_list_mask_kernel), kWordListBlock, 0, 8};
    pl.vsbits = {reinterpret_cast<const void *>(vs_bits_kernel), 64, 0, 32};
    const bool global = V > kVsLdsMaxV || (kn.vs_global.set && kn.vs_global.v != 0);
    pl.vschain = {global ? reinterpret_cast<const void *>(vs_chain_kernel<true>) : reinterpret_cast<const void *>(vs_chain_kernel<false>), kVsBlock,
                  global ? 0 : (int)vs_chain_lds_bytes((V + 31) / 32), 1};
    pl.nzvs.fn = reinterpret_cast<const void *>(nzvs_wave_kernel);
  }
  if (scheme == Scheme::lightpclda) {
    pl.lightpc = {reinterpret_cast<const void *>(lightpc_wave_kernel), 64, (int)light_lds_bytes(K), 0};
// ... 42 lines not shown
```

### ldagroupedgibbssampler_amd/csrc/ggs_host_state.hpp

```cpp
#pragma once
#include <hip/hip_runtime.h>

#include <algorithm>
#include <cctype>
#include <cmath>
#include <cstdio>
#include <cstdlib>
#include <cstring>
#include <new>
#include <string>
#include <vector>

#include "ggs_kernels.hpp"
#include "ggs_z_sliced.hpp"
#include "ggs_z_stream.hpp"
#include "ggs_exact_sum.hpp"
#include "ggs_z_pcgs.hpp"
#include "ggs_z_pcgs_wave.hpp"
#include "ggs_z_collapsed.hpp"
#include "ggs_phi_poisson.hpp"
#include "ggs_alias.hpp"
#include "ggs_z_spalias.hpp"
#include "ggs_z_polyaurn_sparse.hpp"
#include "ggs_phi_vs.hpp"
#include "ggs_z_lightpc.hpp"
#include "ggs_z_lightcollapsed.hpp"
#include "ggs_z_lightpcw2.hpp"
#include "ggs_z_adlda.hpp"
#include "ggs_loglik.hpp"
#include "ggs_heldout.hpp"
#include "ggs_exchange.hpp"
#include "ggs_corpus_lists.hpp"
#include "ggs_distances.hpp"
#include "ggs_topic_summaries.hpp"
#include "ggs_topic_diagnostics.hpp"
#include "ggs_hyper_hist.hpp"

using namespace ggs;

namespace {
const char *debug_env(const char *name) {
  static const bool enabled = [] { const char *e = std::getenv("GGS_DEBUG"); return e && std::atoi(e) == 1; }();
  return enabled ? std::getenv(name) : nullptr;
}
int64_t debug_shrunk(const char *name, int64_t built_in) {
  const char *e = debug_env(name);
  return e ? std::max<int64_t>(1, std::min<int64_t>(built_in, std::atoll(e))) : built_in;
}

struct Knob {
  bool set = false;
  int v = 0;
  double f = 0;
  explicit Knob(const char *name) { if (const char *e = debug_env(name)) { set = true; v = std::atoi(e); f = std::atof(e); } }
  bool is(int x) const { return set && v == x; }
};
struct Knobs {
  Knob zkernel{"GGS_DEBUG_ZKERNEL"}, group{"GGS_DEBUG_GROUP"}, regck{"GGS_DEBUG_REGCK"}, tworows{"GGS_DEBUG_TWOROWS"}, wpc{"GGS_DEBUG_WPC"};
  Knob phi64{"GGS_DEBUG_PHI64"}, split{"GGS_DEBUG_SPLIT"}, hot{"GGS_DEBUG_HOT"}, tile{"GGS_DEBUG_TILE"};
  Knob warm{"GGS_DEBUG_WARM"}, warm_rows{"GGS_DEBUG_WARM_ROWS"}, warm_fill{"GGS_DEBUG_WARM_FILL"}, warm_cpw{"GGS_DEBUG_WARM_CPW"};
  Knob theta_b{"GGS_DEBUG_THETA_B"}, theta_wgs{"GGS_DEBUG_THETA_WGS"}, zparts{"GGS_DEBUG_ZPARTS"}, beside{"GGS_DEBUG_BESIDE"};
  Knob pcgs_wave{"GGS_DEBUG_PCGS_WAVE"}, pcgs_stream{"GGS_DEBUG_PCGS_STREAM"};
  Knob margin{"GGS_DEBUG_MARGIN"}, replays{"GGS_DEBUG_REPLAYS"}, chain{"GGS_DEBUG_CHAIN"}, guided{"GGS_DEBUG_GUIDED"};
  Knob no_overlap{"GGS_DEBUG_NO_OVERLAP"}, theta_main{"GGS_DEBUG_THETA_MAIN"}, gamma_queue{"GGS_DEBUG_GAMMA_QUEUE"};
  Knob num_cus{"GGS_DEBUG_NUM_CUS"}, vs_global{"GGS_DEBUG_VS_GLOBAL"};
};

constexpr int kThetaBlock = 256;

enum class Scheme { ggs, pcgs, collapsed, polyaurn, spalias, lightpclda, polyaurn_sparse, lightcollapsed, nzvsspalias, adlda, lightpcldaw2 };

struct KernelLaunch {
  const void *fn = nullptr;
  int block = 64, lds = 0, per_cu = 0;
};
struct LaunchPlan {
  int32_t kernel = 0;
  bool sliced() const { return kernel == 1; }
  bool stream() const { return kernel >= 2; }
  KernelLaunch z;
  int32_t tile_tokens = 64;
  bool two_rows = false;
  KernelLaunch cold, hot, warm;
  bool f32 = false;
  bool split = true, split_forced = false;
  int32_t wave_lds = 0, ring_base = 0, hot_wave_lds = 0, warm_wave_lds = 0, hot_pitch = 0, Kp32 = 0;
  int32_t hot_cap = 0, warm_cap = 0, warm_docs = 0;
  int32_t warm_tiers_max = 3, warm_min_fill_pct = 40, warm_min_chunks_per_wave = 3;
  struct ZCfg { int32_t parts = 1, z_per_cu = 0, theta_docs = 0, theta_lds = 0, theta_lds_beside_z = 0; } cfg_plain, cfg_parts;
  bool parts_forced = false;
  KernelLaunch theta;
  int32_t theta_docs_main = 0, theta_lds_main = 0;
  KernelLaunch lane, wave, alias, spalias, lightpc, serial, wordlist, pusparse, countalias, lightcol, lightpcw2;
  KernelLaunch vsbits, vschain, wordmask, nzvs;
  KernelLaunch adhead, adlists, adlda;
  KernelLaunch dochist, cellhist;
  bool wave_forced = false;
  int32_t alias_wpb = 0;
  std::vector<const KernelLaunch *> all() const { return {&z, &cold, &hot, &warm, &theta, &lane, &wave, &alias, &spalias, &lightpc, &serial, &wordlist, &pusparse, &countalias, &lightcol, &lightpcw2, &vsbits, &wordmask, &nzvs, &adlda, &dochist, &cellhist}; }
};

enum : uint32_t { kHasAlias = 1, kHasTables = 2, kCountForm = 4, kCountsOnly = 8, kHasWordLists = 16, kDoublySparse = 32, kSparseWalk = 64, kHasMh = 128,
                  kPoissonPhi = 256, kSparseStats = 512, kCountTables = 1024, kNoTheta = 2048 };
struct SchemeRow {
  const char *name;
  int32_t flag, refused;
  int32_t z_kernel;
  KernelLaunch LaunchPlan::*entry;
  size_t (*corpus_lds)(int K, int cap);
  const char *invalid_topic;
  uint32_t caps;
};
constexpr const char *kGgsInvalidTopic = "LDAGroupedGibbsSampler: Topic sampled is invalid!";
constexpr int32_t kModelFlags = GGS_FLAG_COLLAPSED | GGS_FLAG_POLYAURN, kLightFlags = kModelFlags | GGS_FLAG_SPALIAS | GGS_FLAG_LIGHTPCLDA | GGS_FLAG_POLYAURN_SPARSE;
constexpr SchemeRow kSchemes[] = {
    {"ggs", 0, 0, 0, nullptr, nullptr, kGgsInvalidTopic, 0},
    {"pcgs", GGS_FLAG_PCGS, 0, 0, nullptr, nullptr, kGgsInvalidTopic, 0},
    {"collapsed", GGS_FLAG_COLLAPSED, 0, 0, nullptr, nullptr, "SimpleLDA: New topic not sampled." , kCountForm},
    {"polyaurn", GGS_FLAG_POLYAURN, 0, 0, nullptr, nullptr, kGgsInvalidTopic, kPoissonPhi},
    {"spalias", GGS_FLAG_SPALIAS, kModelFlags, 6, &LaunchPlan::spalias, spalias_lds_bytes, kGgsInvalidTopic, kHasAlias | kHasTables | kSparseWalk},
    {"lightpclda", GGS_FLAG_LIGHTPCLDA, kModelFlags | GGS_FLAG_SPALIAS, 7, &LaunchPlan::lightpc, nullptr, kGgsInvalidTopic, kHasAlias | kHasTables | kHasMh},
    {"polyaurn_sparse", GGS_FLAG_POLYAURN_SPARSE, kModelFlags | GGS_FLAG_SPALIAS | GGS_FLAG_LIGHTPCLDA, 8, &LaunchPlan::pusparse, spalias_lds_bytes, kGgsInvalidTopic,
     kHasAlias | kHasTables | kHasWordLists | kDoublySparse | kSparseWalk | kPoissonPhi | kSparseStats},
    {"lightcollapsed", GGS_FLAG_LIGHTCOLLAPSED, kLightFlags | GGS_FLAG_PCGS, 9, &LaunchPlan::lightcol, nullptr, "Collapsed Light-LDA: Sampled invalid topic." ,
     kHasTables | kCountForm | kCountsOnly | kHasWordLists | kHasMh | kCountTables},
    {"nzvsspalias", GGS_FLAG_NZVSSPALIAS, kLightFlags | GGS_FLAG_LIGHTCOLLAPSED, 10, &LaunchPlan::nzvs, spalias_lds_bytes, kGgsInvalidTopic,
     kHasAlias | kHasTables | kHasWordLists | kDoublySparse | kSparseWalk | kSparseStats},
    {"adlda", GGS_FLAG_ADLDA, kLightFlags | GGS_FLAG_PCGS | GGS_FLAG_LIGHTCOLLAPSED | GGS_FLAG_NZVSSPALIAS, 11, &LaunchPlan::adlda, adlda_lds_bytes, "ADLDA: New topic not sampled." ,
     kCountForm | kCountsOnly | kHasWordLists | kSparseStats},
    {"lightpcldaw2", GGS_FLAG_LIGHTPCLDAW2, kLightFlags | GGS_FLAG_LIGHTCOLLAPSED | GGS_FLAG_NZVSSPALIAS | GGS_FLAG_ADLDA, 12, &LaunchPlan::lightpcw2, nullptr,
     "Light PC-LDA (Type topic proposal): Sampled invalid topic." , kHasTables | kHasWordLists | kHasMh | kCountTables | kNoTheta},
};
constexpr int kNumSchemes = (int)(sizeof(kSchemes) / sizeof(kSchemes[0]));
static_assert(kNumSchemes == (int)Scheme::lightpcldaw2 + 1, "one row per Scheme, in the enum's order");
constexpr const SchemeRow &row_of(Scheme s) { return kSchemes[(int)s]; }
constexpr bool has(Scheme s, uint32_t cap) { return (row_of(s).caps & cap) != 0; }
constexpr bool pcgs_family(Scheme s) { return row_of(s).flag != 0; }
constexpr bool has_alias(Scheme s) { return has(s, kHasAlias); }
constexpr bool count_form(Scheme s) { return has(s, kCountForm); }
constexpr bool counts_only(Scheme s) { return has(s, kCountsOnly); }
constexpr bool has_tables(Scheme s) { return has(s, kHasTables); }
constexpr bool has_word_lists(Scheme s) { return has(s, kHasWordLists); }
constexpr bool doubly_sparse(Scheme s) { return has(s, kDoublySparse); }
constexpr bool sparse_walk(Scheme s) { return has(s, kSparseWalk); }
constexpr bool has_mh(Scheme s) { return has(s, kHasMh); }
constexpr bool poisson_phi(Scheme s) { return has(s, kPoissonPhi); }
constexpr bool has_sparse_stats(Scheme s) { return has(s, kSparseStats); }
constexpr bool count_tables(Scheme s) { return has(s, kCountTables); }
constexpr bool no_theta(Scheme s) { return has(s, kNoTheta); }
constexpr bool wave_only(Scheme s) { return row_of(s).entry != nullptr; }
std::string needs_flag(const char *fn, uint32_t cap) {
  std::vector<std::string> names;
  for (const SchemeRow &r : kSchemes)
    if (r.caps & cap) { names.push_back("GGS_FLAG_"); for (const char *c = r.name; *c; ++c) names.back() += (char)std::toupper((unsigned char)*c); }
  std::string msg = std::string(fn) + " needs ";
  for (size_t i = 0; i < names.size(); ++i) msg += (i == 0 ? "" : i + 1 == names.size() ? " or " : ", ") + names[i];
  return msg;
}

constexpr int kEvRing = 8;
struct Events {
  hipEvent_t e[6] = {nullptr, nullptr, nullptr, nullptr, nullptr, nullptr};
  hipEvent_t x[3] = {nullptr, nullptr, nullptr};
  hipEvent_t th0 = nullptr, th1 = nullptr;
  bool used_ahead = false, exchanged = false;
  bool e4_is_e3 = false;
  bool theta_on_main = false;
  bool light = false;
};
}

struct ggs_handle {
  int32_t K = 0, V = 0, Kp = 0, pitch16 = 0, device = 0;
  double beta = 0;
  double beta_sum = 0;
  std::vector<double> alpha;
  uint64_t seed = 0;
  int32_t flags = 0, phi_burn_in = 0, phi_thin = 1;
  Scheme scheme = Scheme::ggs;
  int32_t iteration = 0;
  int32_t n_sampled_phi = 0;

  int64_t D = 0, N = 0, C = 0, S = 0, doc_base = 0, tok_base = 0, global_tokens = -1;
  bool have_corpus = false, have_phi = false, in_sweep = false;
  int32_t num_cus = 0;
  LaunchPlan plan;
  const LaunchPlan::ZCfg *cfg = nullptr;
  int32_t *d_chunk_doc1 = nullptr;
  double margin_scale = 1.0;
  double margin_scale32 = 1.0;

  hipStream_t stream = nullptr;
  int64_t *d_doc_ptr = nullptr, *d_chunk_start = nullptr;
  int32_t *d_tok = nullptr, *d_z = nullptr, *d_chunk_doc = nullptr, *d_chunk_len = nullptr;
  int32_t *d_ct_tok = nullptr, *d_ct_idx = nullptr, *d_ct_ip = nullptr, *d_c_docs = nullptr, *d_hot_words = nullptr;
  int64_t Cs = 0, Cc = 0;
  int32_t *d_order = nullptr;
  int64_t pcgs_order_len = 0;
  bool pcgs_wave = false;
  KernelLaunch pcgs_z;
  int64_t pcgs_items = 0;
  int32_t pa_L = 0;
  double pa_t00 = 0;
  double *d_pa_table = nullptr;
  unsigned long long *d_pa_acc = nullptr;
  bool alias_stale = true;
  double *d_alias_ps = nullptr, *d_alias_tn = nullptr;
  int32_t *d_alias_a = nullptr;
  int32_t sp_cap = 0;
  bool have_priors = false;
  int32_t pr_pitch = 0;
  std::vector<uint32_t> pr_mask;
  uint32_t *d_pr_mask = nullptr;
  double *d_pr_sum_phi = nullptr;
  double *d_pr_pref = nullptr, *d_pr_fn = nullptr;
  double alpha_sum = 0;
  bool alpha_symmetric = false;
  unsigned long long *d_mh = nullptr;
  double *d_ad_den0 = nullptr, *d_ad_s0 = nullptr;
  int32_t *d_tpt = nullptr;
  uint16_t *d_nzw = nullptr;
  int32_t *d_nw = nullptr;
  unsigned long long *d_ps_stats = nullptr;
  double vs_pi = 0.5;
  bool vs_global = false;
  int32_t vs_W = 0, vs_pitch = 0;
  uint32_t *d_vs_cz = nullptr, *d_vs_pz = nullptr, *d_vs_und = nullptr;
  uint32_t *d_vs_mask = nullptr;
  int32_t *d_vs_work = nullptr, *d_vs_s_end = nullptr, *d_vs_rounds = nullptr;
  unsigned long long *d_vs_zero = nullptr;
  enum class VsLists { empty, drawn, nonzero } vs_lists = VsLists::empty;
  bool vs_drawn = false;
  uint64_t *d_lcg = nullptr;
  bool lcg_ready = false;
  int32_t num_hot = 0;
  int32_t *d_perm = nullptr, *d_inv_perm = nullptr, *d_zw = nullptr, *d_seg_word = nullptr, *d_seg_begin = nullptr;
  double *d_theta_next = nullptr;
  hipStream_t side = nullptr;
  hipStream_t side_hot = nullptr;
  hipEvent_t ev_hot_fork = nullptr, ev_hot_join = nullptr;
  bool theta_main = true, chain_on_side = false, theta_main_always = false;
  bool whole_sweep = false;
  hipEvent_t hot_fork_from = nullptr;
  hipEvent_t ev_chain_done = nullptr;
  bool z_split = true, z_split_tried = false;
  int32_t warm_tiers = 0, num_warm = 0, warm_rows_max = 0;
  int64_t Cw = 0, warm_chunks_max = 0;
  int32_t *d_wt_pack = nullptr, *d_w_docs = nullptr, *d_warm_words = nullptr;
  int32_t *d_ht_pack = nullptr, *d_h_docs = nullptr;
  int64_t *d_warm_meta = nullptr;
  bool overlap_theta = true;
  int32_t gamma_queue_cap = 1 << 20;
  std::vector<int64_t> part_doc, part_chunk;
  hipEvent_t ev_part[8] = {nullptr, nullptr, nullptr, nullptr, nullptr, nullptr, nullptr, nullptr};
  int64_t theta_ahead_iter = INT64_MIN;
  float *d_phiT32 = nullptr;
  unsigned long long *d_replays = nullptr;
  int64_t z_f32_launches = 0;
  double *d_alpha = nullptr, *d_theta = nullptr, *d_phiT = nullptr, *d_mag = nullptr, *d_tot = nullptr, *d_phi_mean = nullptr;
  int32_t *d_n_wk = nullptr, *d_n_k = nullptr;
  double *d_sum_pref = nullptr, *d_sum_fn = nullptr;
  int32_t sum_nseg = 0;
  bool exact_sum = true;
  bool sum_guided = true;
  const void *guess_src = nullptr;
  int32_t guess_cols = 0;
  uint32_t *d_status = nullptr;
  int64_t *d_test_ptr = nullptr;
  int32_t *d_test_tok = nullptr, *d_test_docs = nullptr;
  std::vector<int32_t> test_short, test_long, test_huge;
  void *d_heldout_spill = nullptr;
  size_t heldout_spill_bytes = 0;
  double *d_test_ll = nullptr;
  std::vector<int64_t> test_ptr;
  int64_t test_doc_base = 0;
  bool have_test = false;
  void *d_scratch = nullptr;
  size_t scratch_bytes = 0;

  Exchange *xg = nullptr;
  hipStream_t own_stream = nullptr;
  int32_t Ks = 0, Ksm = 0, k0 = 0;
  int64_t *d_koff = nullptr;
  int32_t *d_cnt_send = nullptr, *d_cnt_own = nullptr, *d_cnt_all = nullptr, *d_n_k_own = nullptr;
  double *d_phi_own = nullptr, *d_phi_all0 = nullptr, *d_phi_all1 = nullptr, *d_mag_own = nullptr;
  int32_t *d_krank = nullptr, *d_kcol = nullptr;
  int32_t seg_split = 0, v_split = 0;
  hipStream_t comm_stream = nullptr;
  hipEvent_t ev_half_drawn = nullptr, ev_half_gathered = nullptr;
  int32_t *d_hseg_word = nullptr, *d_hseg_begin = nullptr, *d_hseg_end = nullptr;
  int64_t HS = 0;
  int32_t detail_every = 4;
  bool force_detail = false;
  int64_t sweeps_enqueued = 0;
  bool have_frac = false;
  double frac[5] = {0, 0, 0, 0, 0};
  int32_t count_mode = 0;
  bool counted_sparse = false;
  bool in_group = false;
  int64_t *d_sp_count = nullptr;
  int32_t *d_sp_cnt32 = nullptr, *d_sp_all = nullptr;
  int32_t *d_sp_wg_count = nullptr;
  int64_t *d_sp_wg_off = nullptr;
  int64_t sp_wgs = 0;
  int32_t *d_sp_send = nullptr, *d_sp_recv = nullptr;
  size_t sp_send_cap = 0, sp_recv_cap = 0;
  int64_t sp_pairs_last = 0;
  bool hot_join_pending = false, hot_counted = false;
  bool z_counted = false;
  bool cnt_send_zeroed = false;
  bool z_counts_forced = false;
  bool z_counts = true;
  SliceMap smap{};
  bool counts_global = true;
  bool cnt_own_valid = false;
  bool n_k_valid = false;
  std::vector<ggs_handle *> group;

  std::vector<void **> owned;
  std::vector<hipEvent_t> owned_events;
  std::vector<hipStream_t> owned_streams;
  Events evs[kEvRing];
  int ev_head = 0, ev_pending = 0;
  ggs_timings tm{};
  std::string err;
};

namespace {
int set_err(ggs_handle *h, int code, const std::string &msg) {
  if (h) h->err = msg;
  return code;
}

// ... 103 lines not shown
```

### ldagroupedgibbssampler_amd/csrc/ggs_host_sweep.hpp

```cpp
#pragma once
#include "ggs_host_phi.hpp"

namespace {
int launch_theta(ggs_handle *h, hipStream_t stream, double *dst, int32_t iteration, int64_t d0 = 0, int64_t d1 = -1, int32_t lds = 0, int32_t docs_per_block = 0) {
  if (d1 < 0) d1 = h->D;
  if (d1 <= d0) return GGS_OK;
  if (docs_per_block <= 0) docs_per_block = h->cfg->theta_docs;
  ThetaParams tp{};
  tp.doc_ptr = h->d_doc_ptr + d0; tp.z = h->d_z; tp.alpha = h->d_alpha; tp.theta = dst + (size_t)d0 * h->K; tp.status = h->d_status;
  tp.num_docs = d1 - d0; tp.doc_base = h->doc_base + d0; tp.seed = h->seed; tp.iteration = (uint32_t)iteration;
  tp.K = h->K; tp.docs_per_block = docs_per_block; tp.queue_cap = std::min(kGammaQueue, h->gamma_queue_cap);
  tp.sym_alpha = h->alpha_symmetric ? 1 : 0;
  const int64_t grid = (d1 - d0 + docs_per_block - 1) / docs_per_block;
  void *args[] = {&tp};
  HIP_TRY(h, hipLaunchKernel(h->plan.theta.fn, dim3((unsigned)grid), dim3(kThetaBlock), args, (size_t)(lds ? lds : h->cfg->theta_lds), stream));
  return GGS_OK;
}

int launch_pcgs_z(ggs_handle *h) {
  if (h->N == 0) return GGS_OK;
  PcgsParams pp{};
  pp.tok = h->d_tok; pp.inv_perm = h->d_inv_perm; pp.z = h->d_z; pp.zw = h->d_zw; pp.doc_ptr = h->d_doc_ptr; pp.order = h->d_order;
  pp.alpha = h->d_alpha; pp.phiT = h->d_phiT; pp.status = h->d_status;
  pp.num_docs = h->pcgs_order_len; pp.tok_base = h->tok_base; pp.seed = h->seed; pp.iteration = (uint32_t)h->iteration;
  pp.K = h->K; pp.Kp = h->Kp;
  int rc;
  if (h->alias_stale && (rc = launch_alias_build(h))) return rc;
  if (count_form(h->scheme) || count_tables(h->scheme)) {
    if ((rc = launch_sweep_head(h))) return rc;
    pp.n_wk = h->d_n_wk; pp.n_k = h->d_n_k; pp.beta = h->beta; pp.beta_sum = h->beta_sum;
  }
  PolyaurnSparseParams sp{};
  LightCountParams lp{};
  AdldaParams ad{};
  void *args[] = {&pp, &h->margin_scale};
  if (sparse_walk(h->scheme)) {
    sp.b = pp; sp.ps = h->d_alias_ps; sp.a = h->d_alias_a; sp.type_norm = h->d_alias_tn; sp.cap = h->sp_cap; sp.margin_scale = h->margin_scale;
    sp.nzw = h->d_nzw; sp.nw = h->d_nw; sp.stats = h->d_ps_stats;
    args[0] = static_cast<SpaliasParams *>(&sp);
  } else if (has_mh(h->scheme)) {
    lp.b = pp; lp.ps = h->d_alias_ps; lp.a = h->d_alias_a; lp.mh = h->d_mh; lp.alpha_sum = h->alpha_sum;
    lp.nzw = h->d_nzw; lp.nw = h->d_nw; lp.tpt = h->d_tpt;
    args[0] = static_cast<LightpcParams *>(&lp);
  } else if (h->scheme == Scheme::adlda) {
    ad.b = pp; ad.den0 = h->d_ad_den0; ad.s0 = h->d_ad_s0; ad.nzw = h->d_nzw; ad.nw = h->d_nw; ad.stats = h->d_ps_stats; ad.cap = h->sp_cap; ad.margin_scale = h->margin_scale;
    args[0] = &ad;
  }
  HIP_TRY(h, launch(h, h->pcgs_z, h->pcgs_items, args, h->stream));
  return GGS_OK;
}

bool z_counts_itself(const ggs_handle *h) {
  return h->xg && h->z_counts && h->plan.sliced() && (h->z_counts_forced || h->N <= (int64_t)64 * h->V) && !use_sparse(h);
}
int launch_z(ggs_handle *h, bool force_fused = false, int64_t c0 = 0, int64_t c1 = -1, bool count = false, bool defer_join = false) {
  h->hot_join_pending = false;
  if (h->N == 0) return GGS_OK;
  const LaunchPlan &pl = h->plan;
  ZParams zp{};
  zp.tok = h->d_tok; zp.inv_perm = h->d_inv_perm; zp.z = h->d_z; zp.zw = h->d_zw; zp.chunk_start = h->d_chunk_start; zp.chunk_doc = h->d_chunk_doc; zp.chunk_len = h->d_chunk_len;
  zp.theta = h->d_theta; zp.phiT = h->d_phiT; zp.status = h->d_status;
  zp.tok_base = h->tok_base; zp.seed = h->seed; zp.iteration = (uint32_t)h->iteration;
  zp.K = h->K; zp.Kp = h->Kp; zp.pitch16 = h->pitch16; zp.tile_tokens = pl.tile_tokens;
  zp.margin_scale = h->margin_scale;
  zp.chunk_doc1 = h->d_chunk_doc1; zp.two_rows = (pl.two_rows && h->d_chunk_doc1) ? 1 : 0;
  zp.ct_tok = h->d_ct_tok; zp.ct_idx = h->d_ct_idx; zp.ct_ip = h->d_ct_ip; zp.c_docs = h->d_c_docs; zp.num_cold = h->Cc;
  zp.hot_words = h->d_hot_words; zp.num_hot = h->num_hot; zp.hot_pitch = pl.hot_pitch;
  zp.wave_lds = pl.wave_lds; zp.hot_off = kSlicedWaves * pl.wave_lds; zp.ring_base = pl.ring_base;
  zp.cnt_send = (count && z_counts_itself(h)) ? h->d_cnt_send : nullptr;
  zp.smap = h->smap;
  zp.ht_pack = reinterpret_cast<const int4 *>(h->d_ht_pack); zp.h_docs = h->d_h_docs;
  zp.wt_pack = reinterpret_cast<const int4 *>(h->d_wt_pack); zp.w_docs = h->d_w_docs; zp.warm_words = h->d_warm_words;
  zp.warm_meta = h->d_warm_meta; zp.warm_tiers = h->warm_tiers; zp.warm_rows = pl.warm_cap;
  zp.phiT32 = h->d_phiT32; zp.Kp32 = pl.Kp32; zp.replays = h->d_replays; zp.margin_scale32 = h->margin_scale32;
  void *args[] = {&zp};
  if (!pl.sliced()) {
    if (c1 < 0) c1 = h->C;
    if (c1 <= c0) return GGS_OK;
    zp.chunk_start += c0; zp.chunk_doc += c0; zp.chunk_len += c0; zp.num_chunks = c1 - c0;
    if (zp.chunk_doc1) zp.chunk_doc1 += c0;
    KernelLaunch z = pl.z;
    z.per_cu = h->cfg->z_per_cu;
    HIP_TRY(h, launch(h, z, zp.num_chunks, args, h->stream));
    return GGS_OK;
  }
  zp.num_chunks = h->Cs;
  const int hot_rows_lds = h->num_hot * pl.hot_pitch;
  ZParams wp = zp;
  wp.wave_lds = pl.warm_wave_lds; wp.hot_off = kSlicedWaves * pl.warm_wave_lds;
  void *wargs[] = {&wp};
  auto launch_warm = [&](hipStream_t st) { return h->Cw == 0 ? hipSuccess : launch(h, pl.warm, h->warm_chunks_max, wargs, st, h->warm_rows_max * pl.hot_pitch); };
  if (h->z_split && !force_fused && h->Cs > h->Cc && h->Cc > 0) {
    ZParams hp = zp;
    hp.wave_lds = pl.hot_wave_lds; hp.hot_off = kSlicedWaves * pl.hot_wave_lds;
    void *hargs[] = {&hp};
    if (h->hot_fork_from) {
      HIP_TRY(h, hipStreamWaitEvent(h->side_hot, h->hot_fork_from, 0));
    } else {
      HIP_TRY(h, hipEventRecord(h->ev_hot_fork, h->stream));
      HIP_TRY(h, hipStreamWaitEvent(h->side_hot, h->ev_hot_fork, 0));
    }
    zp.num_chunks = h->Cc; zp.num_hot = 0;
    HIP_TRY(h, launch(h, pl.cold, h->Cc, args, h->stream));
    HIP_TRY(h, launch(h, pl.hot, h->Cs - h->Cc, hargs, h->side_hot, hot_rows_lds));
    HIP_TRY(h, launch_warm(h->side_hot));
    if (defer_join && zp.cnt_send) {
      hipStream_t main_stream = h->stream;
      h->stream = h->side_hot;
      const int rc = launch_count_hot(h);
      h->stream = main_stream;
      if (rc) return rc;
      h->hot_counted = true;
    }
    HIP_TRY(h, hipEventRecord(h->ev_hot_join, h->side_hot));
    if (defer_join) h->hot_join_pending = true;
    else HIP_TRY(h, hipStreamWaitEvent(h->stream, h->ev_hot_join, 0));
  } else {
    HIP_TRY(h, launch(h, pl.cold, std::max(h->Cc, h->Cs - h->Cc), args, h->stream, hot_rows_lds));
    HIP_TRY(h, launch_warm(h->stream));
  }
  if (pl.f32) ++h->z_f32_launches;
  return GGS_OK;
}

bool sample_phi_this_iteration(const ggs_handle *h) {
  return h->phi_burn_in > 0 && h->iteration > h->phi_burn_in && (h->iteration % h->phi_thin) == 0;
}

uint64_t java_lcg_next_ints(int32_t seed, int32_t bound, int64_t n, int32_t *out) {
  constexpr uint64_t kMult = 0x5DEECE66DULL, kMask = (1ULL << 48) - 1;
  uint64_t s = ((uint64_t)(int64_t)seed ^ kMult) & kMask;
  auto next31 = [&]() { s = (s * kMult + 0xBULL) & kMask; return (int32_t)(s >> 17); };
  const int32_t m = bound - 1;
  for (int64_t i = 0; i < n; ++i) {
    int32_t r = next31();
    if ((bound & m) == 0) r = (int32_t)(((int64_t)bound * (int64_t)r) >> 31);
    else
      for (int32_t u = r;; u = next31()) {
        r = u % bound;
        if ((int32_t)((uint32_t)u - (uint32_t)r + (uint32_t)m) >= 0) break;
      }
    out[i] = r;
  }
  return s;
}

int drop_theta_ahead(ggs_handle *h) {
  if (h->side) HIP_TRY(h, hipStreamSynchronize(h->side));
  h->theta_ahead_iter = INT64_MIN;
  return GGS_OK;
}

int settle_sweeps(ggs_handle *h) {
  HIP_TRY(h, hipStreamSynchronize(h->stream));
  for (int j = h->ev_pending - 1; j >= 0; --j) {
    const Events &E = ev_slot(h, j);
    float ms = 0;
    if (E.used_ahead && E.theta_on_main) { HIP_TRY(h, hipEventElapsedTime(&ms, ev_slot(h, j + 1).e[2], E.th1)); }
    else if (E.used_ahead) { HIP_TRY(h, hipEventElapsedTime(&ms, E.th0, E.th1)); }
    else { HIP_TRY(h, hipEventElapsedTime(&ms, E.e[0], E.e[1])); }
    h->tm.theta_ms += ms;
    HIP_TRY(h, hipEventElapsedTime(&ms, E.e[1], E.e[2])); h->tm.z_ms += ms;
    if (E.light) {
      HIP_TRY(h, hipEventElapsedTime(&ms, E.e[2], E.e[5]));
      h->tm.merge_ms += ms * h->frac[0];
      h->tm.exchange_rs_ms += ms * h->frac[1]; h->tm.exchange_ag_ms += ms * h->frac[3]; h->tm.exchange_ms += ms * (h->frac[1] + h->frac[3]);
      h->tm.phi_ms += ms * (h->frac[2] + h->frac[4]);
      h->tm.sweeps += 1;
      h->tm.tokens_sampled += h->N;
      continue;
    }
    HIP_TRY(h, hipEventElapsedTime(&ms, E.e[2], E.e[3])); h->tm.merge_ms += ms;
    if (E.exchanged) {
      float span = 0, part[5] = {ms, 0, 0, 0, 0};
      HIP_TRY(h, hipEventElapsedTime(&part[1], E.e[E.e4_is_e3 ? 3 : 4], E.x[0])); HIP_TRY(h, hipEventElapsedTime(&part[2], E.x[0], E.x[1]));
      HIP_TRY(h, hipEventElapsedTime(&part[3], E.x[1], E.x[2])); HIP_TRY(h, hipEventElapsedTime(&part[4], E.x[2], E.e[5]));
      HIP_TRY(h, hipEventElapsedTime(&span, E.e[2], E.e[5]));
      if (span > 0) {
        const float sum = part[0] + part[1] + part[2] + part[3] + part[4];
        for (int q = 0; q < 5; ++q) h->frac[q] = sum > 0 ? part[q] / sum : 0.0;
        h->have_frac = true;
      }
      h->tm.exchange_ms += part[1]; h->tm.exchange_rs_ms += part[1]; h->tm.phi_ms += part[2];
      h->tm.exchange_ms += part[3]; h->tm.exchange_ag_ms += part[3]; h->tm.phi_ms += part[4];
    } else {
      HIP_TRY(h, hipEventElapsedTime(&ms, E.e[E.e4_is_e3 ? 3 : 4], E.e[5])); h->tm.phi_ms += ms;
    }
// ... 169 lines not shown
```

### ldagroupedgibbssampler_amd/csrc/ggs_layout.hpp

```cpp
#pragma once
#include <stdint.h>

namespace ggs {

constexpr int imax(const int a, const int b) { return a > b ? a : b; }
constexpr int imin(const int a, const int b) { return a < b ? a : b; }
constexpr int round_up(const int x, const int unit) { return (x + unit - 1) / unit * unit; }

constexpr int kMaxLdsBytes = 160 * 1024;
constexpr int kLdsGranule = 2048;
constexpr int lds_alloc_of(const int bytes) { return round_up(bytes, kLdsGranule); }
constexpr int lds_workgroups_per_cu(const int bytes, const int cap) { return imax(1, imin(cap, (kMaxLdsBytes - kLdsGranule) / lds_alloc_of(bytes))); }

constexpr int kSlicedWaves = 4;
constexpr int kChunkDocs = 2;
constexpr int kSlotShift = 30;
constexpr int kWarmMaxTiers = 8;
constexpr int kWarmSlotShift = 16;
constexpr int kWarmDocSlots = 8;
constexpr int kPcgsMaxDocLen = 32767;
constexpr int64_t kSegTokens = 4096;

}
```

### ldagroupedgibbssampler_amd/csrc/ggs_z_kernel.hpp

```cpp
#pragma once
#include "ggs_kernels.hpp"

namespace ggs {

struct SliceMap {
  int32_t rem, size, ksm;
  uint32_t m_size, m_size1;
  int64_t rank_stride;
};
__device__ __forceinline__ int64_t slice_cell(const SliceMap &m, int k, int w) {
  const int cut = m.rem * (m.size + 1);
  int r, c;
  if (k < cut) { r = udiv_small(k, m.m_size1); c = k - r * (m.size + 1); }
  else { const int q = udiv_small(k - cut, m.m_size); r = m.rem + q; c = k - cut - q * m.size; }
  return (int64_t)r * m.rank_stride + (int64_t)w * m.ksm + c;
}

__device__ __forceinline__ void slice_rank_col(const SliceMap &m, int k, int &r, int &c) {
  const int cut = m.rem * (m.size + 1);
  if (k < cut) { r = udiv_small(k, m.m_size1); c = k - r * (m.size + 1); }
  else { const int q = udiv_small(k - cut, m.m_size); r = m.rem + q; c = k - cut - q * m.size; }
}

struct ZParams {
  const int32_t *tok;
  const int32_t *inv_perm;
  int32_t *z;
  int32_t *zw;
  const int64_t *chunk_start;
  const int32_t *chunk_doc;
  const int32_t *chunk_len;
  const double *theta;
  const double *phiT;
  uint32_t *status;
  int64_t num_chunks;
  int64_t tok_base;
  uint64_t seed;
  uint32_t iteration;
  int32_t K, Kp, pitch16, tile_tokens;
  const int32_t *ct_tok;
  const int32_t *ct_idx;
  const int32_t *ct_ip;
  const int32_t *c_docs;
  int64_t num_cold;
  const int32_t *hot_words;
  int32_t num_hot, hot_pitch;
  int32_t hot_off, wave_lds;
  int32_t ring_base;
  double margin_scale;
  const int32_t *chunk_doc1;
  int32_t two_rows;
  int32_t *cnt_send;
  SliceMap smap;
  const int4 *ht_pack;
  const int32_t *h_docs;
  const int4 *wt_pack;
  const int32_t *w_docs;
  const int32_t *warm_words;
  const int64_t *warm_meta;
  int32_t warm_tiers, warm_rows;
  const float *phiT32;
  int32_t Kp32;
  unsigned long long *replays;
  double margin_scale32;
};

struct alignas(16) D2 { double a, b; };

typedef __attribute__((address_space(3))) void lds_void_t;
typedef __attribute__((address_space(1))) const void glb_cvoid_t;
typedef __attribute__((address_space(4))) const int64_t const_i64_t;
typedef __attribute__((address_space(4))) const int32_t const_i32_t;

__device__ __forceinline__ D2 lds_d2(const unsigned char *p) { return *reinterpret_cast<const D2 *>(p); }

constexpr int z_tile_theta_bytes(const int Kp) { return (Kp * 8 + 15) / 16 * 16; }
constexpr int z_tile_lds_bytes(const int Kp, const int pitch16, const int T) { return T * pitch16 * 16 + z_tile_theta_bytes(Kp); }
constexpr int z_tile_rows_in(const int bytes, const int Kp, const int pitch16) { return (bytes - z_tile_theta_bytes(Kp)) / (pitch16 * 16); }

template <int NT>
__global__ __launch_bounds__(64) void z_kernel(ZParams p) {
  extern __shared__ __align__(16) unsigned char smem[];
  const int lane = threadIdx.x;
  const int K = p.K, Kp = p.Kp;
  const int upr = Kp >> 1;
  const int pitch = p.pitch16 * 16;
  unsigned char *thb = smem + (size_t)p.tile_tokens * pitch;
  const unsigned char *phib = reinterpret_cast<const unsigned char *>(p.phiT);
  const size_t rowbytes = (size_t)Kp * 8;
  const const_i64_t *cstart = (const const_i64_t *)p.chunk_start;
  const const_i32_t *clen = (const const_i32_t *)p.chunk_len;
  const const_i32_t *cdoc = (const const_i32_t *)p.chunk_doc;
  const int64_t stride = gridDim.x;
  const int64_t C = p.num_chunks;

  int64_t c = blockIdx.x;
  if (c >= C) return;
  int64_t start = cstart[c];
  int len = clen[c], doc = cdoc[c];
  int64_t nstart = 0;
  int nlen = 0, ndoc = 0;
  if (c + stride < C) { nstart = cstart[c + stride]; nlen = clen[c + stride]; ndoc = cdoc[c + stride]; }
  int w = (lane < len) ? p.tok[start + lane] : 0;
  double tv[NT];
  {
    const double *thg = p.theta + (size_t)doc * K;
#pragma unroll
    for (int t = 0; t < NT; ++t) tv[t] = (t * 64 + lane < K) ? thg[t * 64 + lane] : 0.0;
  }

  for (;;) {
#pragma unroll
    for (int t = 0; t < NT; ++t)
      if (t * 64 + lane < Kp) reinterpret_cast<double *>(thb)[t * 64 + lane] = tv[t];

    const bool has_next = c + stride < C;
    int64_t nnstart = 0;
    int nnlen = 0, nndoc = 0, wn = 0;
    if (has_next) {
      if (c + 2 * stride < C) { nnstart = cstart[c + 2 * stride]; nnlen = clen[c + 2 * stride]; nndoc = cdoc[c + 2 * stride]; }
      wn = (lane < nlen) ? p.tok[nstart + lane] : 0;
      const double *thg = p.theta + (size_t)ndoc * K;
#pragma unroll
      for (int t = 0; t < NT; ++t) tv[t] = (t * 64 + lane < K) ? thg[t * 64 + lane] : 0.0;
    }

    for (int i = 0; i < len; ++i) {
      const int wi = __builtin_amdgcn_readlane(w, i);
      const unsigned char *rb = phib + (size_t)wi * rowbytes;
      unsigned char *dst = smem + (size_t)i * pitch;
      for (int u0 = 0; u0 < upr; u0 += 64) {
        const int u = u0 + lane;
        if (u < upr)
          __builtin_amdgcn_global_load_lds((glb_cvoid_t *)(rb + (size_t)u * 16), (lds_void_t *)(dst + (size_t)u0 * 16), 16, 0, 0);
      }
    }
    asm volatile("s_waitcnt vmcnt(0)");
    __syncthreads();

    if (lane < len) {
      const unsigned char *rowp = smem + lane * pitch;

#define GGS_LD8(A, P) { A##0 = lds_d2(P); A##1 = lds_d2((P) + 16); A##2 = lds_d2((P) + 32); A##3 = lds_d2((P) + 48); }
#define GGS_SUM8(A, S) { \
        sum += (S##0).a * (A##0).a; sum += (S##0).b * (A##0).b; sum += (S##1).a * (A##1).a; sum += (S##1).b * (A##1).b; \
        sum += (S##2).a * (A##2).a; sum += (S##2).b * (A##2).b; sum += (S##3).a * (A##3).a; sum += (S##3).b * (A##3).b; }
      double sum = 0.0;
// ... 88 lines not shown
```

### ldagroupedgibbssampler_amd/csrc/ggs_z_sliced.hpp

```cpp
#pragma once
#include <type_traits>

#include "ggs_slice_ring.hpp"

#ifndef GGS_ABL
#define GGS_ABL 0
#endif

namespace ggs {

constexpr int kSliceTopics = 16;
constexpr int kSlice32Topics = 32;
#ifndef GGS_RING_SLOTS
#define GGS_RING_SLOTS 2
#endif
constexpr int kRingSlots = GGS_RING_SLOTS;
constexpr int kSlicedMaxTopics = 192;
constexpr int kSlicedDefaultTopics = 160;
constexpr int kPhiTailPadBytes = 1024;
constexpr int kHotTailBytes = 64;

constexpr int kWarmThetaPad = 16;
#ifndef GGS_WARM_UNITS
#define GGS_WARM_UNITS 4
#endif
#ifndef GGS_WARM_LANE_DOUBLES
#define GGS_WARM_LANE_DOUBLES 12
#endif
constexpr int warm_docs_for(const int kmax) {
  const int rowd = (kmax + kSliceTopics - 1) / kSliceTopics * kSliceTopics;
  const int d = rowd <= 112 ? GGS_WARM_LANE_DOUBLES / 2 : rowd <= 128 ? GGS_WARM_LANE_DOUBLES / 2 - 1 : 2;
  return d < 2 ? 2 : d > 8 ? 8 : d;
}

constexpr int sliced_kmax(const int K) { return (K + 7) / 8 * 8; }
constexpr int sliced_slices(const int K) { return (sliced_kmax(K) + kSliceTopics - 1) / kSliceTopics; }
constexpr int sliced_ring_base(const int K) { return round_up(imax(kChunkDocs * sliced_kmax(K) * 8, sliced_slices(K) * 128), 256); }
constexpr int sliced_wave_lds(const int K) { return sliced_ring_base(K) + kRingSlots * kSliceBytes; }
constexpr int sliced_cold_lds(const int K) { return kSlicedWaves * sliced_wave_lds(K); }
constexpr int table_row_pitch(const int K) { return sliced_kmax(K) / 8 * 64 + 16; }
constexpr int sliced_fused_lds(const int K, const int rows) { return sliced_cold_lds(K) + rows * table_row_pitch(K); }
constexpr int hot_wave_lds(const int K) { return round_up(kChunkDocs * sliced_slices(K) * kSliceTopics * 8, 256); }
constexpr int warm_wave_lds(const int K) { return round_up(warm_docs_for(sliced_kmax(K)) * (sliced_slices(K) * kSliceTopics * 8 + kWarmThetaPad), 256); }
constexpr int table_lds(const int K, const int wave_lds, const int rows) { return kSlicedWaves * wave_lds + rows * table_row_pitch(K) + kHotTailBytes; }
constexpr int table_rows_beside_cold(const int K, const int wave_lds) {
  return imax(0, imin(255, ((kMaxLdsBytes - lds_alloc_of(sliced_cold_lds(K)) - kSlicedWaves * wave_lds) / kLdsGranule * kLdsGranule - kHotTailBytes) / table_row_pitch(K)));
}
constexpr int table_rows_fused(const int K) { return imax(0, imin(255, (kMaxLdsBytes - sliced_cold_lds(K)) / table_row_pitch(K))); }

struct alignas(8) D2u { double a, b; };

template <int S, int N, class F>
__device__ __forceinline__ void static_for(F &&f) {
  if constexpr (S < N) {
    f(std::integral_constant<int, S>{});
    static_for<S + 1, N>(f);
  }
}

typedef float f2_t __attribute__((ext_vector_type(2)));
typedef float f4_t __attribute__((ext_vector_type(4)));
template <int KMAX>
__device__ __forceinline__ void cold_chunks32(const ZParams &p, unsigned char *thb, unsigned char *ring, const int64_t wid, const int64_t stride, const int lane) {
  constexpr int NS = (KMAX + kSlice32Topics - 1) / kSlice32Topics;
  constexpr int kAhead = NS < kRingSlots - 1 ? NS : kRingSlots - 1;
  constexpr int NT = (KMAX + 63) / 64;
  constexpr int kThetaRow = KMAX * 4;
  const int K = p.K;
  const unsigned char *phib = reinterpret_cast<const unsigned char *>(p.phiT32);
  const size_t rowbytes = (size_t)p.Kp32 * 4;
  const const_i32_t *cdocs = (const const_i32_t *)p.c_docs;
  double *prod = reinterpret_cast<double *>(thb + kChunkDocs * kThetaRow);
  const unsigned char *my_row = ring_lane_row(ring, lane);
  const int rot = ring_lane_rotation(lane);
  const float mscale = (float)p.margin_scale32;

  auto load_theta = [&](const int d0, const int d1, double (&tv)[kChunkDocs][NT]) {
    const double *t0 = p.theta + (size_t)d0 * K, *t1 = p.theta + (size_t)d1 * K;
#pragma unroll
    for (int t = 0; t < NT; ++t) {
      tv[0][t] = (t * 64 + lane < K) ? t0[t * 64 + lane] : 0.0;
      tv[1][t] = (t * 64 + lane < K) ? t1[t * 64 + lane] : 0.0;
    }
  };
  auto stage_theta = [&](const double (&tv)[kChunkDocs][NT]) {
#pragma unroll
    for (int r = 0; r < kChunkDocs; ++r)
#pragma unroll
      for (int t = 0; t < NT; ++t)
        if (t * 64 + lane < KMAX) reinterpret_cast<float *>(thb + r * kThetaRow)[t * 64 + lane] = phi32_of(tv[r][t]);
  };
  auto row_addresses = [&](const int w, const unsigned char *(&ra)[8]) {
    ring_row_addresses(phib, rowbytes, w, (1 << kSlotShift) - 1, lane, ra);
  };
  auto finish = [&](const float (&a)[KMAX], const int64_t c, const int idx, const int ip, const int w) {
    const uint64_t gtok = (uint64_t)(p.tok_base + idx);
    const double U = z_uniform(gtok, p.iteration, p.seed);
    const float A = a[KMAX - 1];
    const float t0 = (float)(U * (double)A);
    const float delta = ((float)(2 * K + 8) * 0x1p-24f * A) * mscale;
    const f2_t nt0 = {-t0, -t0};
    int cnt = 0;
    float m = t0;
    bool live = true;
#pragma unroll
    for (int kb = 0; kb < KMAX; kb += 16) {
      if (live) {
        uint32_t bits = 0;
        float dl = 0.0f;
#pragma unroll
        for (int j = 0; j < 16; j += 2)
          if (kb + j < KMAX) {
            const f2_t d = f2_t{a[kb + j], a[kb + j + 1]} + nt0;
            bits = __builtin_amdgcn_alignbit(bits, __float_as_uint(d.x), 31);
            bits = __builtin_amdgcn_alignbit(bits, __float_as_uint(d.y), 31);
            m = fminf(m, fminf(fabsf(d.x), fabsf(d.y)));
            dl = d.y;
          }
        cnt += __popc(bits);
        live = __any(dl < 0.0f);
      }
    }
    int new_topic = cnt;
    const bool undecided = idx >= 0 && !(A >= 0x1p-60f && A <= 0x1.fffffep127f && m > delta && cnt < K);
    uint64_t pend = __ballot(undecided);
    if (pend) {
// ... 314 lines not shown
      const unsigned char *trow = thb + ((unsigned)w0 >> kSlotShift) * kThetaRow;
      const unsigned char *hrow = smem + p.hot_off + (w0 & ((1 << kSlotShift) - 1)) * p.hot_pitch;

      double sc[KMAX];
      double sum = 0.0;
      if (id0 >= 0) {
        static_for<0, NS>([&](auto sidx) {
          constexpr int s = decltype(sidx)::value;
          D2 ph[kSliceUnits], th[kSliceUnits];
#pragma unroll
          for (int u = 0; u < kSliceUnits; ++u)
            if (s * kSliceTopics + 2 * u + 1 < KMAX) {
              ph[u] = lds_d2(hrow + s * (kSliceTopics * 8) + u * 16);
              th[u] = lds_d2(trow + s * (kSliceTopics * 8) + u * 16);
            }
#pragma unroll
          for (int u = 0; u < kSliceUnits; ++u) {
            constexpr int k0 = s * kSliceTopics;
            const int k = k0 + 2 * u;
            if (k + 1 < KMAX) {
              sc[k] = th[u].a * ph[u].a;
              sum += sc[k];
              sc[k + 1] = th[u].b * ph[u].b;
              sum += sc[k + 1];
            }
          }
        });
      }
      finish(sc, sum, id0, ip0, -1);
      if (!has1) break;
      c += stride;
      w0 = w1; id0 = id1; ip0 = ip1;
#pragma unroll
      for (int r = 0; r < kChunkDocs; ++r)
#pragma unroll
        for (int t = 0; t < NT; ++t) tv0[r][t] = tv1[r][t];
    }
  };

#pragma unroll 1
  for (int phase = 0; phase < 2; ++phase) {
    if ((phase ^ wave) & 1) hot_chunks();
    else if constexpr (F32) cold_chunks32<KMAX>(p, thb, ring, wid, stride, lane);
    else cold_chunks();
  }
}

template <int KMAX>
__global__ __launch_bounds__(kSlicedWaves * 64) void z_sliced_kernel(ZParams p) { z_sliced_body<KMAX, false>(p); }
template <int KMAX>
__global__ __launch_bounds__(kSlicedWaves * 64) void z_sliced32_kernel(ZParams p) { z_sliced_body<KMAX, true>(p); }

template <int KMAX>
__device__ __forceinline__ void load_phi_table(unsigned char *table, const int pitch, const unsigned char *phib, const size_t rowbytes,
                                               const int32_t *words_g, const int nrows, const int wave, const int lane, const int tid) {
  constexpr int upr = KMAX / 2 + 1, kRowsAhead = 6, NP = (upr + 63) / 64;
  const const_i32_t *words = (const const_i32_t *)words_g;
  for (int r0 = wave; r0 < nrows; r0 += kSlicedWaves * kRowsAhead) {
    D2 v[kRowsAhead][NP];
#pragma unroll
    for (int a = 0; a < kRowsAhead; ++a) {
      const int r = r0 + kSlicedWaves * a;
      const unsigned char *src = phib + (size_t)words[r < nrows ? r : r0] * rowbytes;
#pragma unroll
      for (int q = 0; q < NP; ++q) {
        const int u = q * 64 + lane;
        v[a][q] = u < upr - 1 ? *reinterpret_cast<const D2 *>(src + (size_t)u * 16) : D2{0.0, 0.0};
      }
    }
#pragma unroll
    for (int a = 0; a < kRowsAhead; ++a) {
      const int r = r0 + kSlicedWaves * a;
#pragma unroll
      for (int q = 0; q < NP; ++q) {
        const int u = q * 64 + lane;
        if (r < nrows && u < upr) *reinterpret_cast<D2 *>(table + r * pitch + u * 16) = v[a][q];
      }
    }
  }
  if (tid < kHotTailBytes / 8) reinterpret_cast<double *>(table + nrows * pitch)[tid] = 0.0;
}

template <int KMAX, int UB = kSliceUnits>
__device__ __forceinline__ int hot_token(const ZParams &p, const int K, const unsigned char *hrow, const unsigned char *trow, const int id0) {
  constexpr int NS = (KMAX + kSliceTopics - 1) / kSliceTopics;
  double sum = 0.0, ck[NS];
  static_for<0, NS>([&](auto sidx) {
    constexpr int s = decltype(sidx)::value;
#pragma unroll
    for (int b = 0; b < kSliceUnits / UB; ++b) {
      D2 ph[UB], th[UB];
#pragma unroll
      for (int u = 0; u < UB; ++u)
        if (s * kSliceTopics + 2 * (b * UB + u) + 1 < KMAX) {
          ph[u] = lds_d2(hrow + s * (kSliceTopics * 8) + (b * UB + u) * 16);
          th[u] = lds_d2(trow + s * (kSliceTopics * 8) + (b * UB + u) * 16);
        }
#pragma unroll
      for (int u = 0; u < UB; ++u)
        if (s * kSliceTopics + 2 * (b * UB + u) + 1 < KMAX) {
          sum += th[u].a * ph[u].a;
          sum += th[u].b * ph[u].b;
        }
      asm volatile("" : "+v"(sum) : : "memory");
    }
    ck[s] = sum;
  });
  const uint64_t gtok = (uint64_t)(p.tok_base + id0);
  const double t0 = z_uniform(gtok, p.iteration, p.seed) * sum;
  const double delta = (sum * (double)K) * 0x1p-51 * p.margin_scale;
  int gsel = NS;
  static_for<0, NS>([&](auto sidx) {
    constexpr int s = NS - 1 - decltype(sidx)::value;
    if (t0 - ck[s] < -delta) gsel = s;
  });
  bool undecided = gsel == NS;
  if (undecided) gsel = 0;
  double s = 0.0;
  static_for<0, NS - 1>([&](auto sidx) {
    constexpr int q = decltype(sidx)::value;
    if (gsel == q + 1) s = ck[q];
  });
  undecided |= fabs(t0 - s) <= delta;
  int ahead = 0;
  {
    const unsigned char *hs = hrow + gsel * (kSliceTopics * 8), *ts = trow + gsel * (kSliceTopics * 8);
#pragma unroll
    for (int h = 0; h < 2; ++h) {
      D2 ph[kSliceUnits / 2], th[kSliceUnits / 2];
#pragma unroll
      for (int u = 0; u < kSliceUnits / 2; ++u) {
        ph[u] = lds_d2(hs + (h * (kSliceUnits / 2) + u) * 16);
        th[u] = lds_d2(ts + (h * (kSliceUnits / 2) + u) * 16);
      }
#pragma unroll
      for (int u = 0; u < kSliceUnits / 2; ++u) {
        s += th[u].a * ph[u].a;
        double d = t0 - s;
        ahead += d >= -delta;
        undecided |= fabs(d) <= delta;
        s += th[u].b * ph[u].b;
        d = t0 - s;
        ahead += d >= -delta;
        undecided |= fabs(d) <= delta;
      }
      asm volatile("" ::: "memory");
    }
  }
  int new_topic = gsel * kSliceTopics + ahead;
  if (undecided || ahead >= kSliceTopics || new_topic >= K) {
    const double *prow = reinterpret_cast<const double *>(hrow), *trw = reinterpret_cast<const double *>(trow);
    double sample = t0;
    new_topic = -1;
    while (sample > 0.0) {
      ++new_topic;
      if (new_topic >= K) break;
      sample -= trw[new_topic] * prow[new_topic];
    }
    if (new_topic < 0 || new_topic >= K) {
      atomicOr(p.status, ST_INVALID_TOPIC);
      new_topic = new_topic < 0 ? 0 : K - 1;
    }
  }
  return new_topic;
}

typedef int i3v_t __attribute__((ext_vector_type(3)));
typedef int i4v_t __attribute__((ext_vector_type(4)));
template <int N>
__device__ __forceinline__ void wait_vmcnt_take(const i3v_t &e, int &w, int &id, int &ip) {
  asm volatile("s_waitcnt vmcnt(%6)\n\tv_mov_b32 %0, %3\n\tv_mov_b32 %1, %4\n\tv_mov_b32 %2, %5"
               : "=&v"(w), "=&v"(id), "=&v"(ip) : "v"(e.x), "v"(e.y), "v"(e.z), "n"(N) : "memory");
}

template <int KMAX, int DOCS, int PAD, int UB>
__device__ __forceinline__ void table_chunks(const ZParams &p, unsigned char *smem, unsigned char *thb, const int4 *pack, const int32_t *docs_g,
                                             const int64_t first, const int64_t C, const int64_t stride, const int lane, const int32_t *count_words) {
  constexpr int NS = (KMAX + kSliceTopics - 1) / kSliceTopics;
  constexpr int kRowD = NS * kSliceTopics;
  constexpr int kThetaRow = kRowD * 8 + PAD;
  constexpr int NQ = (kRowD + 127) / 128;
  constexpr int kLoads = 1 + DOCS * NQ;
  constexpr int kStores = 2;
  const int K = p.K;
  const const_i32_t *cdocs = (const const_i32_t *)docs_g;
  const uint32_t loff = (uint32_t)lane * 16;
  uint32_t toff[NQ];
#pragma unroll
  for (int q = 0; q < NQ; ++q) { const int k0 = 2 * (q * 64 + lane); toff[q] = (uint32_t)(k0 < K ? k0 : 0) * 8; }
  struct Set { i3v_t e; i4v_t t[DOCS][NQ]; };
  auto issue = [&](const int64_t c, Set &S) {
    typedef int docs8_t __attribute__((ext_vector_type(8)));
    const docs8_t dd = *reinterpret_cast<const __attribute__((address_space(4))) docs8_t *>(cdocs + c * kWarmDocSlots);
    const int4 *lp = pack + c * 64;
    asm volatile("global_load_dwordx3 %0, %1, %2" : "=v"(S.e) : "v"(loff), "s"(lp) : "memory");
#pragma unroll
    for (int r = 0; r < DOCS; ++r) {
      const double *tr = p.theta + (size_t)dd[r] * K;
#pragma unroll
      for (int q = 0; q < NQ; ++q) asm volatile("global_load_dwordx4 %0, %1, %2" : "=v"(S.t[r][q]) : "v"(toff[q]), "s"(tr) : "memory");
    }
  };
  auto arrive = [&](Set &S, const int after, int &w0, int &id0, int &ip0) {
    if (after == 2) wait_vmcnt_take<kLoads + kStores>(S.e, w0, id0, ip0);
    else if (after == 1) wait_vmcnt_take<kLoads>(S.e, w0, id0, ip0);
    else wait_vmcnt_take<0>(S.e, w0, id0, ip0);
#pragma unroll
    for (int r = 0; r < DOCS; ++r)
#pragma unroll
      for (int q = 0; q < NQ; ++q) asm volatile("" : "+v"(S.t[r][q]));
  };
  auto chunk = [&](Set &S, const int64_t c, const int w0, const int id0, const int ip0) {
#pragma unroll
    for (int r = 0; r < DOCS; ++r)
#pragma unroll
      for (int q = 0; q < NQ; ++q)
        if (2 * (q * 64 + lane) < kRowD) {
          const int k0 = 2 * (q * 64 + lane);
          const D2 v = __builtin_bit_cast(D2, S.t[r][q]);
          *reinterpret_cast<D2 *>(thb + r * kThetaRow + k0 * 8) = D2{k0 < K ? v.a : 0.0, k0 + 1 < K ? v.b : 0.0};
        }
    if (c + 2 * stride < C) issue(c + 2 * stride, S);
    const int row = w0 & ((1 << kWarmSlotShift) - 1);
    const unsigned char *trow = thb + ((unsigned)w0 >> kWarmSlotShift) * kThetaRow;
    const unsigned char *hrow = smem + p.hot_off + row * p.hot_pitch;
    if (id0 >= 0) {
      const int new_topic = hot_token<KMAX, UB>(p, K, hrow, trow, id0);
      p.z[id0] = new_topic;
      p.zw[ip0] = new_topic;
      if (count_words)
        __hip_atomic_fetch_add(&p.cnt_send[slice_cell(p.smap, new_topic, count_words[row])], 1, __ATOMIC_RELAXED, __HIP_MEMORY_SCOPE_AGENT);
    }
  };
  int64_t c = first;
  if (c >= C) return;
  Set A, B;
  issue(c, A);
  if (c + stride < C) issue(c + stride, B);
  int done = 0;
  for (;;) {
    int w0, id0, ip0;
    arrive(A, c + stride < C ? (done ? 2 : 1) : 0, w0, id0, ip0);
    chunk(A, c, w0, id0, ip0);
    c += stride;
    if (c >= C) break;
    arrive(B, c + stride < C ? 2 : 0, w0, id0, ip0);
    chunk(B, c, w0, id0, ip0);
    c += stride;
    if (c >= C) break;
    done = 1;
  }
}

template <int KMAX>
__global__ __launch_bounds__(kSlicedWaves * 64) __attribute__((amdgpu_waves_per_eu(4, 4))) void z_hot_kernel(ZParams p) {
  extern __shared__ __align__(16) unsigned char smem[];
  __builtin_amdgcn_s_setprio(3);
  const int lane = threadIdx.x & 63, wave = __builtin_amdgcn_readfirstlane(threadIdx.x >> 6);
  unsigned char *thb = smem + wave * p.wave_lds;
  load_phi_table<KMAX>(smem + p.hot_off, p.hot_pitch, reinterpret_cast<const unsigned char *>(p.phiT), (size_t)p.Kp * 8, p.hot_words, p.num_hot, wave, lane, threadIdx.x);
  __syncthreads();
  table_chunks<KMAX, kChunkDocs, 0, (KMAX <= 128 ? kSliceUnits : kSliceUnits / 2)>(p, smem, thb, p.ht_pack, p.h_docs, (int64_t)blockIdx.x * kSlicedWaves + wave, p.num_chunks - p.num_cold,
                                                 (int64_t)gridDim.x * kSlicedWaves, lane, nullptr);
}


template <int KMAX>
__global__ __launch_bounds__(kSlicedWaves * 64) __attribute__((amdgpu_waves_per_eu(4, 4))) void z_warm_kernel(ZParams p) {
  extern __shared__ __align__(16) unsigned char smem[];
  __builtin_amdgcn_s_setprio(3);
  const int lane = threadIdx.x & 63, wave = __builtin_amdgcn_readfirstlane(threadIdx.x >> 6);
  unsigned char *thb = smem + wave * p.wave_lds;
  const const_i64_t *meta = (const const_i64_t *)p.warm_meta;
  const int64_t stride = (int64_t)gridDim.x * kSlicedWaves;
  const int64_t wid = (int64_t)blockIdx.x * kSlicedWaves + wave;
  for (int tier = 0; tier < p.warm_tiers; ++tier) {
    if (tier) __syncthreads();
    const int32_t *words = p.warm_words + (size_t)tier * p.warm_rows;
    load_phi_table<KMAX>(smem + p.hot_off, p.hot_pitch, reinterpret_cast<const unsigned char *>(p.phiT), (size_t)p.Kp * 8, words, (int)meta[p.warm_tiers + 1 + tier], wave, lane, threadIdx.x);
    __syncthreads();
    table_chunks<KMAX, warm_docs_for(KMAX), kWarmThetaPad, GGS_WARM_UNITS>(p, smem, thb, p.wt_pack, p.w_docs, meta[tier] + wid, meta[tier + 1], stride, lane,
                                                                          p.cnt_send ? words : nullptr);
  }
}

}
```

### ldagroupedgibbssampler_amd/native.py

```python
import ctypes as C

import numpy as np

from . import _lib

OK = 0
ERR_NEGATIVE_COUNT, ERR_INVALID_TOPIC, ERR_RNG_EXHAUSTED, ERR_BAD_ARG = 1, 2, 3, 4
ERR_HIP, ERR_STATE, ERR_UNSUPPORTED, ERR_INVARIANT = 5, 6, 7, 8
FLAG_PARANOID, FLAG_SAVE_PHI_MEAN, FLAG_PCGS, FLAG_COLLAPSED, FLAG_POLYAURN, FLAG_SPALIAS, FLAG_LIGHTPCLDA = 1, 2, 4, 8, 16, 32, 64
FLAG_POLYAURN_SPARSE = 128
FLAG_LIGHTCOLLAPSED = 256
FLAG_NZVSSPALIAS = 512
FLAG_ADLDA = 1024
FLAG_LIGHTPCLDAW2 = 2048
SCHEME_FLAGS = {"ggs": 0, "pcgs": FLAG_PCGS, "collapsed": FLAG_COLLAPSED, "polyaurn": FLAG_POLYAURN, "spalias": FLAG_SPALIAS, "lightpclda": FLAG_LIGHTPCLDA,
                "polyaurn_sparse": FLAG_POLYAURN_SPARSE, "lightcollapsed": FLAG_LIGHTCOLLAPSED, "nzvsspalias": FLAG_NZVSSPALIAS, "adlda": FLAG_ADLDA}
PURPOSE_Z, PURPOSE_THETA, PURPOSE_PHI, PURPOSE_INIT_PHI = 1, 2, 3, 4
TOP_KINDS = {"top": 0, "relevance": 1, "distinctive": 2, "salient": 3, "k1": 4}
TOP_WORDS_MAX = 128
TOPIC_DIAGNOSTIC_NAMES = ("tokens", "document_entropy", "word-length", "coherence", "uniform_dist", "corpus_dist", "eff_num_words", "token-doc-diff",
                          "rank_1_docs", "allocation_ratio", "allocation_count")
TOPIC_SCORE_ROWS = tuple(x for x in TOPIC_DIAGNOSTIC_NAMES if x != "word-length")
TOPIC_WORD_SCORE_ROWS = ("coherence", "uniform_dist", "corpus_dist", "token-doc-diff")

# ... 359 lines not shown
            if other.ndim != 2 or other.shape[1] != self.K:
                raise ValueError("other must be [n][K]")
            op, n = _dp(other), other.shape[0]
        self._chk(self._L.ggs_min_doc_distances(self._h, op, n, _dp(out)))
        return out

    def min_topic_distance(self):
        v = C.c_double()
        self._chk(self._L.ggs_min_topic_distance(self._h, C.byref(v)))
        return v.value

    def top_words(self, kind, n, lam=0.6, scores=False):
        idx = np.empty((self.K, int(n)), np.int32)
        sc = np.empty((self.K, int(n)), np.float64) if scores else None
        self._chk(self._L.ggs_top_words(self._h, _top_kind(kind), int(n), float(lam), _ip(idx), _dp(sc) if scores else None))
        return (idx, sc) if scores else idx

    def top_words_phases(self, kind, n, lam=0.6, element_chain=False):
        ms = np.zeros(4, np.float64)
        self._chk(self._L.ggs_debug_top_words_phases(self._h, _top_kind(kind), int(n), float(lam), int(bool(element_chain)), _dp(ms)))
        return dict(zip(("mass_k", "total", "words", "select_merge"), ms.tolist()))

    def topic_doc_statistics(self, n, idx=None, clogc_in=None):
        n = int(n)
        if idx is not None:
            idx = np.ascontiguousarray(idx, np.int32)
            if idx.shape != (self.K, n):
                raise ValueError("idx must be [K][n]")
        if clogc_in is not None:
            clogc_in = np.ascontiguousarray(clogc_in, np.float64)
            if clogc_in.shape != (self.K,):
                raise ValueError("clogc_in must be [K]")
        m = max(n, 0)
        codoc, stats, clogc = np.empty((self.K, m, m), np.int32), np.empty((self.K, 9), np.int32), np.empty(self.K, np.float64)
        self._chk(self._L.ggs_topic_doc_statistics(self._h, n, _ip(idx) if idx is not None else None, _dp(clogc_in) if clogc_in is not None else None,
                                                   _ip(codoc), _ip(stats), _dp(clogc)))
        return codoc, stats, clogc

    def topic_scores(self, n, idx, codoc, doc_stats, clogc, word_scores=False):
        n = int(n)
        m = max(n, 0)
        idx, codoc = np.ascontiguousarray(idx, np.int32), np.ascontiguousarray(codoc, np.int32)
        doc_stats, clogc = np.ascontiguousarray(doc_stats, np.int32), np.ascontiguousarray(clogc, np.float64)
        if idx.shape != (self.K, m) or codoc.shape != (self.K, m, m) or doc_stats.shape != (self.K, 9) or clogc.shape != (self.K,):
            raise ValueError("idx [K][n], codoc [K][n][n], doc_stats [K][9], clogc [K]")
        ts = np.empty((len(TOPIC_SCORE_ROWS), self.K), np.float64)
        ws = np.empty((len(TOPIC_WORD_SCORE_ROWS), self.K, m), np.float64) if word_scores else None
        self._chk(self._L.ggs_topic_scores(self._h, n, _ip(idx), _ip(codoc), _ip(doc_stats), _dp(clogc), _dp(ts), _dp(ws) if word_scores else None))
        return (ts, ws) if word_scores else ts

    def topic_diagnostics(self, n, alphabet=None):
        idx = self.top_words("top", n)
        codoc, stats, clogc = self.topic_doc_statistics(n, idx)
        ts, ws = self.topic_scores(n, idx, codoc, stats, clogc, word_scores=True)
        return TopicDiagnostics(idx, codoc, stats, clogc, ts, ws, alphabet)

    def topic_diagnostics_phases(self, n):
        ms = np.zeros(7, np.float64)
        self._chk(self._L.ggs_debug_topic_diagnostics_phases(self._h, int(n), _dp(ms)))
        return dict(zip(("membership", "document_pass", "column_statistics", "clogc_chain", "totals", "sort_and_sorted_chains", "small_scores"), ms.tolist()))

    def set_test_corpus(self, doc_ptr, tokens, doc_base=0):
        doc_ptr = np.ascontiguousarray(doc_ptr, np.int64)
        tokens = np.ascontiguousarray(tokens, np.int32)
        self._test_docs = doc_ptr.size - 1
        self._chk(self._L.ggs_set_test_corpus(self._h, self._test_docs, doc_ptr.ctypes.data_as(C.POINTER(C.c_int64)),
                                              tokens.ctypes.data_as(C.POINTER(C.c_int32)), int(doc_base)))

    def heldout_log_likelihood(self, num_particles=100):
        doc_ll = np.zeros(getattr(self, "_test_docs", 0), np.float64)
        tot = C.c_double()
        self._chk(self._L.ggs_heldout_log_likelihood(self._h, int(num_particles), doc_ll.ctypes.data_as(C.POINTER(C.c_double)), C.byref(tot)))
        return tot.value, doc_ll

    def launch_info(self):
        c, l, b, nh, zp = C.c_int64(), C.c_int32(), C.c_int32(), C.c_int32(), C.c_int32()
        self._chk(self._L.ggs_get_launch_info(self._h, C.byref(c), C.byref(l), C.byref(b)))
        self._chk(self._L.ggs_get_num_hot_words(self._h, C.byref(nh)))
        self._chk(self._L.ggs_get_z_parts(self._h, C.byref(zp)))
        zk, zf, zc = C.c_int32(), C.c_int32(), C.c_int32()
        self._chk(self._L.ggs_get_z_form(self._h, C.byref(zk), C.byref(zf), C.byref(zc)))
        wt, ww, wd = C.c_int32(), C.c_int32(), C.c_int32()
        self._chk(self._L.ggs_get_warm_tiers(self._h, C.byref(wt), C.byref(ww), C.byref(wd)))
        return {"num_chunks": c.value, "lds_bytes_z": l.value, "docs_per_block_theta": b.value, "num_hot": nh.value, "z_parts": zp.value,
                "warm_tiers": wt.value, "num_warm": ww.value, "warm_docs_per_chunk": wd.value,
                "z_kernel": Z_KERNEL_NAMES.get(zk.value, str(zk.value)) + (" + z_warm_kernel (%d tiers)" % wt.value if wt.value else ""), "z_form": {0: "n/a", 1: "split", 2: "fused"}.get(zf.value, str(zf.value)),
                "z_form_calibrated": bool(zc.value)}


Z_KERNEL_NAMES = {0: "z_kernel (whole-row tiles)", 1: "z_sliced_kernel + z_hot_kernel (score registers)", 2: "z_stream1_kernel (one pass)",
                  3: "z_stream_kernel (two passes)", 4: "pcgs_sliced_kernel (lane per document)", 5: "pcgs_wave_kernel (wave per document)",
                  6: "spalias_wave_kernel (wave per document)", 7: "lightpc_wave_kernel (wave per document)",
                  8: "polyaurn_sparse_wave_kernel (wave per document)", 9: "lightcollapsed_wave_kernel (wave per document)",
                  10: "nzvs_wave_kernel (wave per document)", 11: "adlda_wave_kernel (wave per document)", 12: "lightpcw2_wave_kernel (wave per document)"}


class GGSGroup:

    @classmethod
    def adopt(cls, handles):
        self = cls.__new__(cls)
        self._L = _lib.load()
        n = len(handles)
        self._arr = (C.c_void_p * n)(*[h._h for h in handles])
        self.handles, self._owns = list(handles), False
        self._chk(self._L.ggs_group_adopt(self._arr, n))
        return self

    def __init__(self, num_topics, num_types, alpha, beta, seed, device_ids, flags=0, phi_burn_in=0, phi_mean_thin=1, alias_poisson_threshold=0):
        self._L = _lib.load()
        self._owns = True
        _lib.share_rccl_with_torch()
        cfg, keep = _make_config(num_topics, num_types, alpha, beta, seed, 0, flags, phi_burn_in, phi_mean_thin, alias_poisson_threshold)
        n = len(device_ids)
        devs = (C.c_int32 * n)(*[int(d) for d in device_ids])
        self._arr = (C.c_void_p * n)()
        rc = self._L.ggs_group_create(C.byref(cfg), n, devs, self._arr)
        if rc:
            raise GGSError(rc, "ggs_group_create failed")
        self.handles = [GGSHandle(num_topics, num_types, alpha, beta, seed, _adopt=C.c_void_p(self._arr[i])) for i in range(n)]

    def _chk(self, rc):
        if rc:
            msgs = [self._L.ggs_last_error(h._h).decode() for h in self.handles]
            raise GGSError(rc, next((m for m in msgs if m), ""))

    def set_z(self, z_list, redraw_phi=True):
        zs = [np.ascontiguousarray(z, np.int32) for z in z_list]
        ptrs = (C.POINTER(C.c_int32) * len(zs))(*[_ip(z) for z in zs])
        self._chk(self._L.ggs_group_set_z(self._arr, len(zs), ptrs, int(bool(redraw_phi))))

    def sweep(self, n=1):
        self._chk(self._L.ggs_group_sweep(self._arr, len(self.handles), int(n)))

    def gather_counts(self):
        self._chk(self._L.ggs_group_gather_counts(self._arr, len(self.handles)))

    def close(self):
        if getattr(self, "handles", None):
            if getattr(self, "_owns", True):
                for h in self.handles:
                    h._h = None
                self._L.ggs_group_destroy(self._arr, len(self.handles))
            self.handles = []

    def __del__(self):
        try:
            self.close()
        except Exception:
            pass


def learn_symmetric_concentration(count_hist, obs_lengths, num_dimensions, current):
    ch, ol = np.ascontiguousarray(count_hist, np.int32), np.ascontiguousarray(obs_lengths, np.int32)
    out = C.c_double()
    rc = _lib.load().ggs_learn_symmetric_concentration(_ip(ch), ch.size, _ip(ol), ol.size, int(num_dimensions), float(current), C.byref(out))
    if rc:
        raise GGSError(rc, "ggs_learn_symmetric_concentration: bad argument")
    return out.value


def learn_parameters(params, obs, obs_lengths, shape=1.001, scale=1.0, iterations=1):
    if not (isinstance(params, np.ndarray) and params.dtype == np.float64 and params.flags.c_contiguous and params.ndim == 1):
        raise ValueError("params must be a contiguous float64 vector: it is updated in place")
    ob, ol = np.ascontiguousarray(obs, np.int32), np.ascontiguousarray(obs_lengths, np.int32)
    if ob.ndim != 2 or ob.shape[0] != params.size:
        raise ValueError("obs must be [K][n_bins]")
    out = C.c_double()
    rc = _lib.load().ggs_learn_parameters(_dp(params), params.size, _ip(ob), ob.shape[1], _ip(ol), ol.size, float(shape), float(scale), int(iterations),
# ... 200 lines not shown
```

Before: 17130.

## Share hot-word cumulative scores across repeated (doc, word) pairs in a new pairs kernel

Adds a z_pairs_kernel that groups hot-word tokens by (document, word) pair. It computes the cumulative topic-score prefix once per pair into LDS, then reuses it for every token of that pair. Only the per-token uniform draw and search remain per token. Host-side list construction builds the pair chunks, and the kernel is enabled by default in split mode. In exchange it adds LDS per wave, which can shrink hot table capacity, and it adds preprocessing plus another token ordering.

After: 17500 (median of 6 runs). 1.02x the previous value.

```diff
diff --git a/include/ggs_hip.h b/include/ggs_hip.h
--- a/include/ggs_hip.h
+++ b/include/ggs_hip.h
@@ -153,6 +153,7 @@
 int ggs_get_warm_tiers(ggs_handle *h, int32_t *tiers, int32_t *warm_words, int32_t *docs_per_chunk);
 int ggs_get_z_parts(ggs_handle *h, int32_t *parts);
 int ggs_get_z_form(ggs_handle *h, int32_t *kernel, int32_t *form, int32_t *calibrated);
+int ggs_get_hot_pairs(ggs_handle *h, int32_t *enabled, int64_t *pair_chunks, int64_t *pairs, int64_t *tokens);
 int ggs_debug_philox(int32_t device_id, int64_t n, const uint32_t *ctr , const uint32_t *key , uint32_t *out );
 int ggs_debug_math(int32_t device_id, int32_t op , int64_t n, const double *x, const double *y, double *out);
 int ggs_debug_draw(int32_t device_id, int32_t kind , uint64_t seed, uint32_t iteration,
diff --git a/ldagroupedgibbssampler_amd/_lib.py b/ldagroupedgibbssampler_amd/_lib.py
--- a/ldagroupedgibbssampler_amd/_lib.py
+++ b/ldagroupedgibbssampler_amd/_lib.py
@@ -104,6 +104,7 @@
     "ggs_get_z_parts": (C.c_int, [_vp, _ip]),
     "ggs_get_z_form": (C.c_int, [_vp, _ip, _ip, _ip]),
     "ggs_get_warm_tiers": (C.c_int, [_vp, _ip, _ip, _ip]),
+    "ggs_get_hot_pairs": (C.c_int, [_vp, _ip, _lp, _lp, _lp]),
     "ggs_attach_exchange": (C.c_int, [_vp, C.c_int32, C.c_int32, C.POINTER(GGSExchangeOps)]),
     "ggs_rccl_unique_id": (C.c_int, [_vp]),
     "ggs_attach_rccl": (C.c_int, [_vp, C.c_int32, C.c_int32, _vp]),
diff --git a/ldagroupedgibbssampler_amd/csrc/ggs_api.hip b/ldagroupedgibbssampler_amd/csrc/ggs_api.hip
--- a/ldagroupedgibbssampler_amd/csrc/ggs_api.hip
+++ b/ldagroupedgibbssampler_amd/csrc/ggs_api.hip
@@ -173,6 +173,7 @@
   shape.pcgs = pcgs; shape.sliced = pl.sliced(); shape.two_rows = pl.two_rows;
   shape.hot_cap = pl.hot_cap; shape.warm_cap = pl.warm_cap; shape.warm_docs = pl.warm_docs;
   shape.warm_tiers_max = pl.warm_tiers_max; shape.warm_min_fill_pct = pl.warm_min_fill_pct; shape.warm_min_chunks_per_wave = pl.warm_min_chunks_per_wave;
+  shape.hot_pairs = pl.hot_pairs;
   shape.sliced_waves = (int64_t)h->num_cus * kSlicedWaves; shape.pcgs_waves = (int64_t)h->num_cus * pl.lane.per_cu;
   const CorpusLists L = build_corpus_lists(shape, D, doc_ptr, tokens);
   if (pcgs) {
@@ -191,7 +192,8 @@
   h->part_doc = L.part_doc; h->part_chunk = L.part_chunk;
   h->pcgs_order_len = (int64_t)L.order.size();
   h->num_hot = (int32_t)L.hot_words.size(); h->HS = (int64_t)L.hseg_word.size();
-  h->Cc = L.Cc; h->Cs = L.Cs;
+  h->Cc = L.Cc; h->Cs = L.Cs; h->Cp = L.Cp; h->hp_pairs = h->hp_tokens = 0;
+  for (int64_t c = 0; c < L.Cp; ++c) { h->hp_pairs += L.hp_docs[(size_t)(c * kWarmDocSlots + kHotPairCountSlot)]; h->hp_tokens += L.hp_docs[(size_t)(c * kWarmDocSlots + kHotPairTokSlot)]; }
   h->warm_tiers = L.warm_tiers; h->num_warm = L.num_warm; h->Cw = L.Cw; h->warm_chunks_max = L.warm_chunks_max; h->warm_rows_max = L.warm_rows_max;
 
   const size_t theta_elems = (size_t)D * h->K + 2;
@@ -208,6 +210,7 @@
   if (h->C && ((rc = upload(h, &h->d_chunk_start, L.cstart)) || (rc = upload(h, &h->d_chunk_doc, L.cdoc)) || (rc = upload(h, &h->d_chunk_len, L.clen)) ||
                (pl.two_rows && (rc = upload(h, &h->d_chunk_doc1, L.cdoc1)))))
     return rc;
+  if (L.Cp > 0 && ((rc = upload(h, &h->d_hp_pair, L.hp_pair)) || (rc = upload(h, &h->d_hp_docs, L.hp_docs)) || (rc = upload(h, &h->d_hp_tok, L.hp_tok)))) return rc;
   if (L.warm_tiers > 0 && ((rc = upload(h, &h->d_wt_pack, L.wt_pack)) || (rc = upload(h, &h->d_w_docs, L.w_docs)) ||
                            (rc = upload(h, &h->d_warm_words, L.warm_words)) || (rc = upload(h, &h->d_warm_meta, L.warm_meta))))
     return rc;
@@ -1141,6 +1144,16 @@
   if (tiers) *tiers = on ? h->warm_tiers : 0;
   if (warm_words) *warm_words = on ? h->num_warm : 0;
   if (docs_per_chunk) *docs_per_chunk = on && h->warm_tiers ? h->plan.warm_docs : 0;
+  return GGS_OK;
+}
+
+int ggs_get_hot_pairs(ggs_handle *h, int32_t *enabled, int64_t *pair_chunks, int64_t *pairs, int64_t *tokens) {
+  if (!h) return GGS_ERR_BAD_ARG;
+  const bool built = h->have_corpus && h->plan.sliced() && h->plan.hot_pairs;
+  if (enabled) *enabled = (built && h->Cp > 0 && h->z_split && h->Cs > h->Cc && h->Cc > 0) ? 1 : 0;
+  if (pair_chunks) *pair_chunks = built ? h->Cp : 0;
+  if (pairs) *pairs = built ? h->hp_pairs : 0;
+  if (tokens) *tokens = built ? h->hp_tokens : 0;
   return GGS_OK;
 }
 
diff --git a/ldagroupedgibbssampler_amd/csrc/ggs_corpus_lists.hpp b/ldagroupedgibbssampler_amd/csrc/ggs_corpus_lists.hpp
--- a/ldagroupedgibbssampler_amd/csrc/ggs_corpus_lists.hpp
+++ b/ldagroupedgibbssampler_amd/csrc/ggs_corpus_lists.hpp
@@ -18,6 +18,7 @@
   int32_t z_parts = 1;
   int32_t hot_cap = 0, warm_cap = 0, warm_docs = 0;
   int32_t warm_tiers_max = 0, warm_min_fill_pct = 0, warm_min_chunks_per_wave = 0;
+  bool hot_pairs = false;
   int64_t sliced_waves = 0;
   int64_t pcgs_waves = 0;
 };
@@ -37,6 +38,8 @@
   int64_t Cw = 0, warm_chunks_max = 0;
   std::vector<int32_t> wt_pack, w_docs, warm_words;
   std::vector<int64_t> warm_meta;
+  std::vector<int32_t> hp_pair, hp_docs, hp_tok;
+  int64_t Cp = 0;
 };
 
 namespace lists_detail {
@@ -176,6 +179,55 @@
   return pack;
 }
 
+inline void hot_pair_lists(const int64_t D, const int64_t *doc_ptr, const int32_t *tokens, const std::vector<int32_t> &row_of, CorpusLists &L) {
+  std::vector<std::pair<int32_t, int32_t>> dt;
+  std::vector<int32_t> ctok;
+  int npairs = 0, ndocs = 0, ntok = 0, last = -1;
+  bool open = false;
+  auto close_chunk = [&]() {
+    if (!open) return;
+    int32_t *meta = &L.hp_docs[L.hp_docs.size() - (size_t)kWarmDocSlots];
+    meta[kHotPairTokSlot] = ntok; meta[kHotPairCountSlot] = npairs; meta[kHotPairRoundSlot] = (int32_t)(L.hp_tok.size() / (4 * 64));
+    L.hp_tok.insert(L.hp_tok.end(), ctok.begin(), ctok.end());
+    for (int j = ntok; j % 64 != 0; ++j) { const int32_t idle[4] = {0, -1, 0, 0}; L.hp_tok.insert(L.hp_tok.end(), idle, idle + 4); }
+    ctok.clear();
+    open = false;
+  };
+  for (int64_t d = 0; d < D; ++d) {
+    dt.clear();
+    for (int64_t i = doc_ptr[d]; i < doc_ptr[d + 1]; ++i)
+      if (row_of[(size_t)tokens[i]] >= 0) dt.push_back({row_of[(size_t)tokens[i]], (int32_t)i});
+    std::sort(dt.begin(), dt.end());
+    for (size_t a = 0; a < dt.size();) {
+      size_t b = a;
+      while (b < dt.size() && dt[b].first == dt[a].first) ++b;
+      for (; a < b; a += (size_t)kHotPairTokenCap) {
+        const int m = (int)std::min<size_t>(b - a, (size_t)kHotPairTokenCap);
+        if (!open || npairs == 64 || ntok + m > kHotPairTokenCap || ((int32_t)d != last && ndocs == kHotPairDocs)) {
+          close_chunk();
+          L.hp_pair.resize(L.hp_pair.size() + 64, 0);
+          L.hp_docs.insert(L.hp_docs.end(), (size_t)kWarmDocSlots, 0);
+          for (int r = 0; r < kHotPairDocs; ++r) L.hp_docs[L.hp_docs.size() - (size_t)kWarmDocSlots + (size_t)r] = (int32_t)d;
+          open = true; npairs = 0; ndocs = 1; ntok = 0; last = (int32_t)d;
+        } else if ((int32_t)d != last) {
+          L.hp_docs[L.hp_docs.size() - (size_t)kWarmDocSlots + (size_t)ndocs] = (int32_t)d; ++ndocs; last = (int32_t)d;
+        }
+        const int32_t word = dt[a].first | ((ndocs - 1) << kWarmSlotShift);
+        L.hp_pair[L.hp_pair.size() - 64 + (size_t)npairs] = word;
+        for (int j = 0; j < m; ++j) {
+          const int32_t i = dt[a + (size_t)j].second;
+          const int32_t e[4] = {word | (npairs << kHotPairLaneShift), i, L.inv[(size_t)i], 0};
+          ctok.insert(ctok.end(), e, e + 4);
+        }
+        ++npairs; ntok += m;
+      }
+      a = b;
+    }
+  }
+  close_chunk();
+  L.Cp = (int64_t)(L.hp_pair.size() / 64);
+}
+
 inline void sliced_lists(const CorpusShape &s, const int64_t D, const int64_t *doc_ptr, const int32_t *tokens, std::vector<int32_t> warm_cand, CorpusLists &L) {
   ChunkBuilder cold, hot;
   std::vector<int32_t> row_of((size_t)s.V, -1);
@@ -207,6 +259,7 @@
       if (r >= 0) hot.add(r, (int32_t)i, (int32_t)d);
       else if (r == -1) cold.add(tokens[i], (int32_t)i, (int32_t)d);
     }
+  if (s.hot_pairs) hot_pair_lists(D, doc_ptr, tokens, row_of, L);
   cold.sort_lanes();
   hot.sort_lanes();
   for (ChunkBuilder &b : warm) b.sort_lanes();
diff --git a/ldagroupedgibbssampler_amd/csrc/ggs_host_plan.hpp b/ldagroupedgibbssampler_amd/csrc/ggs_host_plan.hpp
--- a/ldagroupedgibbssampler_amd/csrc/ggs_host_plan.hpp
+++ b/ldagroupedgibbssampler_amd/csrc/ggs_host_plan.hpp
@@ -22,6 +22,7 @@
 
 const void *hot_kernel_for(int K) { GGS_KMAX_SWITCH(z_hot_kernel) }
 const void *warm_kernel_for(int K) { GGS_KMAX_SWITCH(z_warm_kernel) }
+const void *pairs_kernel_for(int K) { GGS_KMAX_SWITCH(z_pairs_kernel) }
 const void *pcgs_kernel_for(int K) { GGS_KMAX_SWITCH(pcgs_sliced_kernel) }
 const void *polyaurn_kernel_for(int K) { GGS_KMAX_SWITCH(polyaurn_sliced_kernel) }
 const void *collapsed_kernel_for(int K) {
@@ -102,10 +103,13 @@
       pl.ring_base = sliced_ring_base(K); pl.wave_lds = sliced_wave_lds(K); pl.hot_pitch = table_row_pitch(K);
       pl.hot_wave_lds = hot_wave_lds(K); pl.warm_wave_lds = warm_wave_lds(K);
       if (kn.split.set) { pl.split = kn.split.v != 0; pl.split_forced = kn.split.v == 2; }
-      pl.hot_cap = pl.split ? table_rows_beside_cold(K, pl.hot_wave_lds) : table_rows_fused(K);
+      pl.hot_pairs = pl.split && !kn.hot_pairs.is(0);
+      pl.pairs_wave_lds = pairs_wave_lds(K);
+      pl.hot_cap = !pl.split ? table_rows_fused(K) : table_rows_beside_cold(K, pl.hot_pairs ? std::max(pl.hot_wave_lds, pl.pairs_wave_lds) : pl.hot_wave_lds);
       if (kn.hot.set) pl.hot_cap = std::max(0, std::min(pl.hot_cap, kn.hot.v));
       pl.cold = {pl.f32 ? sliced32_kernel_for(K) : sliced_kernel_for(K), kSlicedWaves * 64, sliced_cold_lds(K), 1};
       pl.hot = {hot_kernel_for(K), kSlicedWaves * 64, table_lds(K, pl.hot_wave_lds, 0), 1};
+      if (pl.hot_pairs) pl.pairs = {pairs_kernel_for(K), kSlicedWaves * 64, table_lds(K, pl.pairs_wave_lds, 0), 1};
       pl.warm = {warm_kernel_for(K), kSlicedWaves * 64, table_lds(K, pl.warm_wave_lds, 0), 1};
       pl.warm_docs = warm_docs_for(sliced_kmax(K));
       pl.warm_cap = table_rows_beside_cold(K, pl.warm_wave_lds);
diff --git a/ldagroupedgibbssampler_amd/csrc/ggs_host_state.hpp b/ldagroupedgibbssampler_amd/csrc/ggs_host_state.hpp
--- a/ldagroupedgibbssampler_amd/csrc/ggs_host_state.hpp
+++ b/ldagroupedgibbssampler_amd/csrc/ggs_host_state.hpp
@@ -58,7 +58,7 @@
 struct Knobs {
   Knob zkernel{"GGS_DEBUG_ZKERNEL"}, group{"GGS_DEBUG_GROUP"}, regck{"GGS_DEBUG_REGCK"}, tworows{"GGS_DEBUG_TWOROWS"}, wpc{"GGS_DEBUG_WPC"};
   Knob phi64{"GGS_DEBUG_PHI64"}, split{"GGS_DEBUG_SPLIT"}, hot{"GGS_DEBUG_HOT"}, tile{"GGS_DEBUG_TILE"};
-  Knob warm{"GGS_DEBUG_WARM"}, warm_rows{"GGS_DEBUG_WARM_ROWS"}, warm_fill{"GGS_DEBUG_WARM_FILL"}, warm_cpw{"GGS_DEBUG_WARM_CPW"};
+  Knob hot_pairs{"GGS_DEBUG_HOT_PAIRS"}, warm{"GGS_DEBUG_WARM"}, warm_rows{"GGS_DEBUG_WARM_ROWS"}, warm_fill{"GGS_DEBUG_WARM_FILL"}, warm_cpw{"GGS_DEBUG_WARM_CPW"};
   Knob theta_b{"GGS_DEBUG_THETA_B"}, theta_wgs{"GGS_DEBUG_THETA_WGS"}, zparts{"GGS_DEBUG_ZPARTS"}, beside{"GGS_DEBUG_BESIDE"};
   Knob pcgs_wave{"GGS_DEBUG_PCGS_WAVE"}, pcgs_stream{"GGS_DEBUG_PCGS_STREAM"};
   Knob margin{"GGS_DEBUG_MARGIN"}, replays{"GGS_DEBUG_REPLAYS"}, chain{"GGS_DEBUG_CHAIN"}, guided{"GGS_DEBUG_GUIDED"};
@@ -82,6 +82,9 @@
   int32_t tile_tokens = 64;
   bool two_rows = false;
   KernelLaunch cold, hot, warm;
+  KernelLaunch pairs;
+  bool hot_pairs = false;
+  int32_t pairs_wave_lds = 0;
   bool f32 = false;
   bool split = true, split_forced = false;
   int32_t wave_lds = 0, ring_base = 0, hot_wave_lds = 0, warm_wave_lds = 0, hot_pitch = 0, Kp32 = 0;
@@ -97,7 +100,7 @@
   KernelLaunch dochist, cellhist;
   bool wave_forced = false;
   int32_t alias_wpb = 0;
-  std::vector<const KernelLaunch *> all() const { return {&z, &cold, &hot, &warm, &theta, &lane, &wave, &alias, &spalias, &lightpc, &serial, &wordlist, &pusparse, &countalias, &lightcol, &lightpcw2, &vsbits, &wordmask, &nzvs, &adlda, &dochist, &cellhist}; }
+  std::vector<const KernelLaunch *> all() const { return {&z, &cold, &hot, &pairs, &warm, &theta, &lane, &wave, &alias, &spalias, &lightpc, &serial, &wordlist, &pusparse, &countalias, &lightcol, &lightpcw2, &vsbits, &wordmask, &nzvs, &adlda, &dochist, &cellhist}; }
 };
 
 enum : uint32_t { kHasAlias = 1, kHasTables = 2, kCountForm = 4, kCountsOnly = 8, kHasWordLists = 16, kDoublySparse = 32, kSparseWalk = 64, kHasMh = 128,
@@ -249,6 +252,8 @@
   int32_t *d_wt_pack = nullptr, *d_w_docs = nullptr, *d_warm_words = nullptr;
   int32_t *d_ht_pack = nullptr, *d_h_docs = nullptr;
   int64_t *d_warm_meta = nullptr;
+  int32_t *d_hp_pair = nullptr, *d_hp_docs = nullptr, *d_hp_tok = nullptr;
+  int64_t Cp = 0, hp_pairs = 0, hp_tokens = 0;
   bool overlap_theta = true;
   int32_t gamma_queue_cap = 1 << 20;
   std::vector<int64_t> part_doc, part_chunk;
diff --git a/ldagroupedgibbssampler_amd/csrc/ggs_host_sweep.hpp b/ldagroupedgibbssampler_amd/csrc/ggs_host_sweep.hpp
--- a/ldagroupedgibbssampler_amd/csrc/ggs_host_sweep.hpp
+++ b/ldagroupedgibbssampler_amd/csrc/ggs_host_sweep.hpp
@@ -102,7 +102,13 @@
     }
     zp.num_chunks = h->Cc; zp.num_hot = 0;
     HIP_TRY(h, launch(h, pl.cold, h->Cc, args, h->stream));
-    HIP_TRY(h, launch(h, pl.hot, h->Cs - h->Cc, hargs, h->side_hot, hot_rows_lds));
+    if (pl.hot_pairs && h->Cp > 0) {
+      hp.wave_lds = pl.pairs_wave_lds; hp.hot_off = kSlicedWaves * pl.pairs_wave_lds;
+      hp.hp_pair = h->d_hp_pair; hp.hp_docs = h->d_hp_docs; hp.hp_tok = reinterpret_cast<const int4 *>(h->d_hp_tok); hp.num_pair_chunks = h->Cp;
+      HIP_TRY(h, launch(h, pl.pairs, h->Cp, hargs, h->side_hot, hot_rows_lds));
+    } else {
+      HIP_TRY(h, launch(h, pl.hot, h->Cs - h->Cc, hargs, h->side_hot, hot_rows_lds));
+    }
     HIP_TRY(h, launch_warm(h->side_hot));
     if (defer_join && zp.cnt_send) {
       hipStream_t main_stream = h->stream;
diff --git a/ldagroupedgibbssampler_amd/csrc/ggs_layout.hpp b/ldagroupedgibbssampler_amd/csrc/ggs_layout.hpp
--- a/ldagroupedgibbssampler_amd/csrc/ggs_layout.hpp
+++ b/ldagroupedgibbssampler_amd/csrc/ggs_layout.hpp
@@ -18,6 +18,11 @@
 constexpr int kWarmMaxTiers = 8;
 constexpr int kWarmSlotShift = 16;
 constexpr int kWarmDocSlots = 8;
+constexpr int kHotPairDocs = 2;
+constexpr int kHotPairRounds = 4;
+constexpr int kHotPairTokenCap = 64 * kHotPairRounds;
+constexpr int kHotPairLaneShift = 24;
+constexpr int kHotPairTokSlot = 4, kHotPairCountSlot = 5, kHotPairRoundSlot = 6;
 constexpr int kPcgsMaxDocLen = 32767;
 constexpr int64_t kSegTokens = 4096;
 
diff --git a/ldagroupedgibbssampler_amd/csrc/ggs_z_kernel.hpp b/ldagroupedgibbssampler_amd/csrc/ggs_z_kernel.hpp
--- a/ldagroupedgibbssampler_amd/csrc/ggs_z_kernel.hpp
+++ b/ldagroupedgibbssampler_amd/csrc/ggs_z_kernel.hpp
@@ -63,6 +63,10 @@
   int32_t Kp32;
   unsigned long long *replays;
   double margin_scale32;
+  const int32_t *hp_pair;
+  const int32_t *hp_docs;
+  const int4 *hp_tok;
+  int64_t num_pair_chunks;
 };
 
 struct alignas(16) D2 { double a, b; };
diff --git a/ldagroupedgibbssampler_amd/csrc/ggs_z_sliced.hpp b/ldagroupedgibbssampler_amd/csrc/ggs_z_sliced.hpp
--- a/ldagroupedgibbssampler_amd/csrc/ggs_z_sliced.hpp
+++ b/ldagroupedgibbssampler_amd/csrc/ggs_z_sliced.hpp
@@ -42,6 +42,8 @@
 constexpr int sliced_fused_lds(const int K, const int rows) { return sliced_cold_lds(K) + rows * table_row_pitch(K); }
 constexpr int hot_wave_lds(const int K) { return round_up(kChunkDocs * sliced_slices(K) * kSliceTopics * 8, 256); }
 constexpr int warm_wave_lds(const int K) { return round_up(warm_docs_for(sliced_kmax(K)) * (sliced_slices(K) * kSliceTopics * 8 + kWarmThetaPad), 256); }
+constexpr int pairs_record_pitch(const int K) { return (sliced_slices(K) | 1) * 8; }
+constexpr int pairs_wave_lds(const int K) { return round_up(kHotPairDocs * sliced_slices(K) * kSliceTopics * 8 + 64 * pairs_record_pitch(K), 256); }
 constexpr int table_lds(const int K, const int wave_lds, const int rows) { return kSlicedWaves * wave_lds + rows * table_row_pitch(K) + kHotTailBytes; }
 constexpr int table_rows_beside_cold(const int K, const int wave_lds) {
   return imax(0, imin(255, ((kMaxLdsBytes - lds_alloc_of(sliced_cold_lds(K)) - kSlicedWaves * wave_lds) / kLdsGranule * kLdsGranule - kHotTailBytes) / table_row_pitch(K)));
@@ -522,9 +524,9 @@
 }
 
 template <int KMAX, int UB = kSliceUnits>
-__device__ __forceinline__ int hot_token(const ZParams &p, const int K, const unsigned char *hrow, const unsigned char *trow, const int id0) {
+__device__ __forceinline__ void hot_pass1(const unsigned char *hrow, const unsigned char *trow, double (&ck)[(KMAX + kSliceTopics - 1) / kSliceTopics]) {
   constexpr int NS = (KMAX + kSliceTopics - 1) / kSliceTopics;
-  double sum = 0.0, ck[NS];
+  double sum = 0.0;
   static_for<0, NS>([&](auto sidx) {
     constexpr int s = decltype(sidx)::value;
 #pragma unroll
@@ -546,6 +548,12 @@
     }
     ck[s] = sum;
   });
+}
+template <int KMAX>
+__device__ __forceinline__ int hot_decide(const ZParams &p, const int K, const unsigned char *hrow, const unsigned char *trow, const int id0,
+                                          const double (&ck)[(KMAX + kSliceTopics - 1) / kSliceTopics]) {
+  constexpr int NS = (KMAX + kSliceTopics - 1) / kSliceTopics;
+  const double sum = ck[NS - 1];
   const uint64_t gtok = (uint64_t)(p.tok_base + id0);
   const double t0 = z_uniform(gtok, p.iteration, p.seed) * sum;
   const double delta = (sum * (double)K) * 0x1p-51 * p.margin_scale;
@@ -604,6 +612,12 @@
   }
   return new_topic;
 }
+template <int KMAX, int UB = kSliceUnits>
+__device__ __forceinline__ int hot_token(const ZParams &p, const int K, const unsigned char *hrow, const unsigned char *trow, const int id0) {
+  double ck[(KMAX + kSliceTopics - 1) / kSliceTopics];
+  hot_pass1<KMAX, UB>(hrow, trow, ck);
+  return hot_decide<KMAX>(p, K, hrow, trow, id0, ck);
+}
 
 typedef int i3v_t __attribute__((ext_vector_type(3)));
 typedef int i4v_t __attribute__((ext_vector_type(4)));
@@ -724,4 +738,110 @@
   }
 }
 
-}
+template <int KMAX>
+__global__ __launch_bounds__(kSlicedWaves * 64) __attribute__((amdgpu_waves_per_eu(4, 4))) void z_pairs_kernel(ZParams p) {
+  constexpr int NS = (KMAX + kSliceTopics - 1) / kSliceTopics;
+  constexpr int kRowD = NS * kSliceTopics, kThetaRow = kRowD * 8, NQ = (kRowD + 127) / 128;
+  constexpr int kRec = (NS | 1) * 8;
+  constexpr int R = kHotPairRounds;
+  constexpr int UB = kSliceUnits / 2;
+  extern __shared__ __align__(16) unsigned char smem[];
+  __builtin_amdgcn_s_setprio(3);
+  const int lane = threadIdx.x & 63, wave = __builtin_amdgcn_readfirstlane(threadIdx.x >> 6);
+  unsigned char *thb = smem + wave * p.wave_lds;
+  unsigned char *rec = thb + kHotPairDocs * kThetaRow;
+  load_phi_table<KMAX>(smem + p.hot_off, p.hot_pitch, reinterpret_cast<const unsigned char *>(p.phiT), (size_t)p.Kp * 8, p.hot_words, p.num_hot, wave, lane, threadIdx.x);
+  __syncthreads();
+  const int K = p.K;
+  const int64_t C = p.num_pair_chunks, stride = (int64_t)gridDim.x * kSlicedWaves;
+  int64_t c = (int64_t)blockIdx.x * kSlicedWaves + wave;
+  if (c >= C) return;
+  const const_i32_t *cdocs = (const const_i32_t *)p.hp_docs;
+  uint32_t toff[NQ];
+#pragma unroll
+  for (int q = 0; q < NQ; ++q) { const int k0 = 2 * (q * 64 + lane); toff[q] = (uint32_t)(k0 < K ? k0 : 0) * 8; }
+
+  typedef i4v_t i4v8_t __attribute__((aligned(8)));
+  struct Set { int pw, nt; i3v_t e[R]; i4v_t t[kHotPairDocs][NQ]; };
+  auto fetch = [&](const int64_t cc, Set &S) {
+    typedef int docs8_t __attribute__((ext_vector_type(8)));
+    const docs8_t dd = *reinterpret_cast<const __attribute__((address_space(4))) docs8_t *>(cdocs + cc * kWarmDocSlots);
+    S.nt = dd[kHotPairTokSlot];
+    S.pw = p.hp_pair[cc * 64 + lane];
+    const int4 *tp = p.hp_tok + ((int64_t)dd[kHotPairRoundSlot] * 64 + lane);
+#pragma unroll
+    for (int r = 0; r < R; ++r) {
+      if (r * 64 < S.nt) S.e[r] = *reinterpret_cast<const i3v_t *>(tp + r * 64);
+      else S.e[r] = i3v_t{0, -1, 0};
+    }
+#pragma unroll
+    for (int r = 0; r < kHotPairDocs; ++r)
+#pragma unroll
+      for (int q = 0; q < NQ; ++q)
+        S.t[r][q] = *reinterpret_cast<const i4v8_t *>(reinterpret_cast<const unsigned char *>(p.theta + (size_t)dd[r] * K) + toff[q]);
+  };
+
+  Set N;
+  fetch(c, N);
+  i3v_t ce[R];
+  int res[R];
+#pragma unroll
+  for (int r = 0; r < R; ++r) { ce[r] = i3v_t{0, -1, 0}; res[r] = 0; }
+  for (;;) {
+    asm volatile("" : "+v"(N.pw));
+#pragma unroll
+    for (int r = 0; r < R; ++r) asm volatile("" : "+v"(N.e[r]));
+#pragma unroll
+    for (int r = 0; r < kHotPairDocs; ++r)
+#pragma unroll
+      for (int q = 0; q < NQ; ++q) asm volatile("" : "+v"(N.t[r][q]));
+#pragma unroll
+    for (int r = 0; r < kHotPairDocs; ++r)
+#pragma unroll
+      for (int q = 0; q < NQ; ++q)
+        if (2 * (q * 64 + lane) < kRowD) {
+          const int k0 = 2 * (q * 64 + lane);
+          const D2 v = __builtin_bit_cast(D2, N.t[r][q]);
+          *reinterpret_cast<D2 *>(thb + r * kThetaRow + k0 * 8) = D2{k0 < K ? v.a : 0.0, k0 + 1 < K ? v.b : 0.0};
+        }
+    asm volatile("" ::: "memory");
+#pragma unroll
+    for (int r = 0; r < R; ++r)
+      if (ce[r].y >= 0) { p.z[ce[r].y] = res[r]; p.zw[ce[r].z] = res[r]; }
+    const int pw = N.pw, nt = N.nt;
+#pragma unroll
+    for (int r = 0; r < R; ++r) ce[r] = N.e[r];
+    const bool has1 = c + stride < C;
+    if (has1) fetch(c + stride, N);
+    asm volatile("" ::: "memory");
+    {
+      const unsigned char *hrow = smem + p.hot_off + (pw & ((1 << kWarmSlotShift) - 1)) * p.hot_pitch;
+      const unsigned char *trow = thb + ((unsigned)pw >> kWarmSlotShift) * kThetaRow;
+      double ck[NS];
+      hot_pass1<KMAX, UB>(hrow, trow, ck);
+#pragma unroll
+      for (int s = 0; s < NS; ++s) reinterpret_cast<double *>(rec + lane * kRec)[s] = ck[s];
+    }
+    asm volatile("s_waitcnt lgkmcnt(0)" ::: "memory");
+#pragma unroll
+    for (int r = 0; r < R; ++r)
+      if (r * 64 < nt && ce[r].y >= 0) {
+        const int w = ce[r].x;
+        const unsigned char *hrow = smem + p.hot_off + (w & ((1 << kWarmSlotShift) - 1)) * p.hot_pitch;
+        const unsigned char *trow = thb + (((unsigned)w >> kWarmSlotShift) & ((1 << (kHotPairLaneShift - kWarmSlotShift)) - 1)) * kThetaRow;
+        const double *rk = reinterpret_cast<const double *>(rec + ((unsigned)w >> kHotPairLaneShift) * kRec);
+        double ck[NS];
+#pragma unroll
+        for (int s = 0; s < NS; ++s) ck[s] = rk[s];
+        res[r] = hot_decide<KMAX>(p, K, hrow, trow, ce[r].y, ck);
+      }
+    asm volatile("s_waitcnt lgkmcnt(0)" ::: "memory");
+    if (!has1) break;
+    c += stride;
+  }
+#pragma unroll
+  for (int r = 0; r < R; ++r)
+    if (ce[r].y >= 0) { p.z[ce[r].y] = res[r]; p.zw[ce[r].z] = res[r]; }
+}
+
+}
diff --git a/ldagroupedgibbssampler_amd/native.py b/ldagroupedgibbssampler_amd/native.py
--- a/ldagroupedgibbssampler_amd/native.py
+++ b/ldagroupedgibbssampler_amd/native.py
@@ -465,9 +465,13 @@
         self._chk(self._L.ggs_get_z_form(self._h, C.byref(zk), C.byref(zf), C.byref(zc)))
         wt, ww, wd = C.c_int32(), C.c_int32(), C.c_int32()
         self._chk(self._L.ggs_get_warm_tiers(self._h, C.byref(wt), C.byref(ww), C.byref(wd)))
+        hp, hc, hn, ht = C.c_int32(), C.c_int64(), C.c_int64(), C.c_int64()
+        self._chk(self._L.ggs_get_hot_pairs(self._h, C.byref(hp), C.byref(hc), C.byref(hn), C.byref(ht)))
+        zname = "z_sliced_kernel + z_pairs_kernel (score registers)" if zk.value == 1 and hp.value else Z_KERNEL_NAMES.get(zk.value, str(zk.value))
         return {"num_chunks": c.value, "lds_bytes_z": l.value, "docs_per_block_theta": b.value, "num_hot": nh.value, "z_parts": zp.value,
                 "warm_tiers": wt.value, "num_warm": ww.value, "warm_docs_per_chunk": wd.value,
-                "z_kernel": Z_KERNEL_NAMES.get(zk.value, str(zk.value)) + (" + z_warm_kernel (%d tiers)" % wt.value if wt.value else ""), "z_form": {0: "n/a", 1: "split", 2: "fused"}.get(zf.value, str(zf.value)),
+                "hot_pairs": bool(hp.value), "hot_pair_chunks": hc.value, "hot_pairs_per_token": (hn.value / ht.value) if ht.value else 0.0,
+                "z_kernel": zname + (" + z_warm_kernel (%d tiers)" % wt.value if wt.value else ""), "z_form": {0: "n/a", 1: "split", 2: "fused"}.get(zf.value, str(zf.value)),
                 "z_form_calibrated": bool(zc.value)}
 
 
```
